# getreu/stringsext

Measured on AMD Instinct MI355X. Metric: GiB/s scanned, higher is better.
Workload: dtype u8

## Files before the change

include/stringsext_amd.h:

```cpp
#ifndef STRINGSEXT_AMD_H
#define STRINGSEXT_AMD_H
#include <stddef.h>
#include <stdint.h>

#ifdef __cplusplus
extern "C" {
#endif

#define SX_ABI_VERSION 4

enum {
    SX_OK = 0,
    SX_E_INVALID = -1,
    SX_E_NO_DEVICE = -2,
    SX_E_HIP = -3,
    SX_E_NOMEM = -4,
    SX_E_STATE = -5,
    SX_E_HALO = -6
};

enum {
    SX_ENC_X_USER_DEFINED = 0, SX_ENC_UTF8 = 1, SX_ENC_UTF16LE = 2, SX_ENC_UTF16BE = 3,
    SX_ENC_KOI8_R = 16, SX_ENC_IBM866 = 17, SX_ENC_ISO_8859_2 = 18, SX_ENC_ISO_8859_5 = 19,
    SX_ENC_ISO_8859_15 = 20, SX_ENC_WINDOWS_1251 = 21, SX_ENC_WINDOWS_1252 = 22,
// ... 171 lines not shown
                         sx_result** out, uint64_t* end_pos);
int sx_scan_shard(sx_ctx* ctx, const uint8_t* bytes, uint64_t buf_off, uint64_t buf_len,
                  uint64_t own_lo, uint64_t own_hi, const uint64_t* start_at,
                  uint64_t file_stream_off, int input_file_id, int reuse_runs,
                  sx_result** out, uint64_t* end_pos);
int sx_replay_shard_runs(sx_ctx* ctx, const uint8_t* bytes, uint64_t buf_off, uint64_t buf_len,
                         uint64_t own_lo, uint64_t own_hi, const uint64_t* start_at,
                         uint64_t file_stream_off, int input_file_id,
                         const sx_run* const* runs, const uint64_t* n_runs,
                         sx_result** out, uint64_t* end_pos);

typedef int (*sx_allgather_fn)(void* user, const void* send, uint64_t bytes, void* recv);
typedef int (*sx_shard_buffer_fn)(void* user, uint64_t lo, uint64_t hi, const void** ptr, int* is_device);
typedef int (*sx_shard_runs_fn)(void* user, const uint8_t* bytes, uint64_t buf_off, uint64_t buf_len,
                                const sx_run* const** runs, const uint64_t** n_runs);
void sx_shard_bounds(uint64_t file_len, int world, int rank, uint64_t* own_lo, uint64_t* own_hi);
int sx_scan_sharded(sx_ctx* ctx, int rank, int world, uint64_t file_len, uint64_t file_stream_off, int input_file_id,
                    uint64_t halo, sx_shard_buffer_fn get_buffer, void* buffer_user, sx_shard_runs_fn get_runs, void* runs_user,
                    sx_allgather_fn allgather, void* allgather_user, sx_result** out, uint64_t* counts, uint64_t* overflow);
int sx_shard_splice(const sx_finding* const* findings, const uint64_t* n_findings, const uint8_t* const* arenas,
                    const uint64_t* arena_lens, int world, uint64_t file_len, sx_result** out);
int sx_shard_splice_segs(const sx_finding* const* findings, const uint64_t* n_findings, const uint8_t* const* arenas,
                         const uint64_t* arena_lens, const uint32_t* n_segs_of_rank, int world, uint64_t file_len, sx_result** out);

#define SX_TRANSPORT_ID_BYTES 128
typedef struct sx_transport sx_transport;
int  sx_transport_rccl_id(uint8_t* id128);
int  sx_transport_rccl_create(sx_transport** out, int hip_device, int rank, int world, const uint8_t* id128);
void sx_transport_destroy(sx_transport* t);
const char* sx_transport_last_error(const sx_transport* t);
int  sx_transport_allgather(void* transport, const void* send, uint64_t bytes, void* recv);
int  sx_transport_gather(sx_transport* t, const sx_result* mine, int root, uint64_t file_len, sx_result** out);

int               sx_result_segment_device(const sx_result* r, uint64_t i, const void** d_records, uint64_t* n_findings,
                                           const uint8_t** d_arena, uint64_t* arena_len, int* packed, sx_segment_info* info);
uint64_t          sx_result_count(const sx_result* r);
uint64_t          sx_result_segments(const sx_result* r);
int               sx_result_segment(const sx_result* r, uint64_t index, const sx_finding** findings,
                                    uint64_t* n_findings, const uint8_t** arena, uint64_t* arena_len);
int               sx_result_segment_packed(const sx_result* r, uint64_t index, const void** findings, uint64_t* n_findings,
                                           const uint8_t** arena, uint64_t* arena_len, int* packed, sx_segment_info* info);
const sx_finding* sx_result_findings(const sx_result* r);
const uint8_t*    sx_result_arena(const sx_result* r, uint64_t* len);
void              sx_result_free(sx_result* r);

#define SX_OUTPUT_BOM "\xEF\xBB\xBF"
int sx_print_findings(const sx_ctx* ctx, const sx_result* r, int n_inputs, int radix,
                      int no_metadata, uint8_t** out, uint64_t* out_len);
int sx_print_findings_device(sx_ctx* ctx, const sx_result* r, int n_inputs, int radix, int no_metadata,
                             const uint8_t** d_text, uint64_t* text_len);

#define SX_SELECT_MAX_PATTERNS 16
#define SX_SELECT_MAX_PATTERN_BYTES 64
enum { SX_SELECT_ASCII_NOCASE = 1u,
       SX_SELECT_INVERT = 2u };
typedef struct sx_pattern { const uint8_t* bytes; uint32_t len; } sx_pattern;
int sx_result_select_device(sx_ctx* ctx, const sx_result* r, const sx_pattern* patterns, int n_patterns,
                            uint32_t flags, sx_result** out);

#define SX_SELECT_SET_MAX_PATTERNS      65536u
#define SX_SELECT_SET_MAX_PATTERN_BYTES 255u
#define SX_SELECT_SET_MAX_TOTAL_BYTES   (1u << 20)
typedef struct sx_select_set sx_select_set;
typedef struct sx_select_set_info {
    uint32_t n_patterns, states, classes, nocase;
    uint64_t table_bytes;
    uint32_t lds_states;
    uint32_t reserved;
} sx_select_set_info;
int  sx_select_set_create(sx_ctx* ctx, const sx_pattern* patterns, uint32_t n_patterns, uint32_t flags, sx_select_set** out);
int  sx_select_set_info_get(const sx_select_set* set, sx_select_set_info* out);
void sx_select_set_free(sx_select_set* set);
int  sx_result_select_set_device(sx_ctx* ctx, const sx_result* r, const sx_select_set* set, uint32_t flags, sx_result** out);

int  sx_get_stats(const sx_ctx* ctx, sx_stats* out);
void sx_free(void* p);

int sx_fill_background_device(sx_ctx* ctx, void* device_bytes, uint64_t first_byte_index,
                              uint64_t len, uint64_t seed);
int sx_device_alloc(sx_ctx* ctx, uint64_t bytes, void** device_ptr);
int sx_device_free(sx_ctx* ctx, void* device_ptr);
int sx_device_upload(sx_ctx* ctx, void* device_dst, const void* host_src, uint64_t bytes);
int sx_device_download(sx_ctx* ctx, void* host_dst, const void* device_src, uint64_t bytes);
int sx_device_read_bandwidth(sx_ctx* ctx, const void* device_bytes, uint64_t len, int repeats,
                             double* gbytes_per_s);

#ifdef __cplusplus
}
#endif
#endif
```

stringsext_amd/__init__.py:

```python
import ctypes as C
import os

_HERE = os.path.dirname(os.path.abspath(__file__))
LIB_PATH = os.environ.get("SX_LIB") or os.path.join(_HERE, "libstringsext_amd.so")

SX_OK, SX_E_INVALID, SX_E_NO_DEVICE, SX_E_HIP, SX_E_NOMEM, SX_E_STATE, SX_E_HALO = 0, -1, -2, -3, -4, -5, -6
SX_HOST_ONLY = -1
SX_OPT_GENERIC_KERNELS, SX_OPT_DEVICE_REPLAY, SX_OPT_HOST_REPLAY = 1, 2, 4
SX_OPT_NO_FUSED_SCAN = 64
SX_SELECT_MAX_PATTERNS, SX_SELECT_MAX_PATTERN_BYTES = 16, 64
SX_SELECT_ASCII_NOCASE, SX_SELECT_INVERT = 1, 2
SX_SELECT_SET_MAX_PATTERNS, SX_SELECT_SET_MAX_PATTERN_BYTES, SX_SELECT_SET_MAX_TOTAL_BYTES = 65536, 255, 1 << 20
SX_OPT_RESULT_ON_DEVICE = 32
ENC = {"x-user-defined": 0, "utf-8": 1, "utf-16le": 2, "utf-16be": 3, "koi8-r": 16, "ibm866": 17,
       "iso-8859-2": 18, "iso-8859-5": 19, "iso-8859-15": 20, "windows-1251": 21, "windows-1252": 22,
       "iso-8859-3": 23, "iso-8859-4": 24, "iso-8859-6": 25, "iso-8859-7": 26, "iso-8859-8": 27,
       "iso-8859-8-i": 28, "iso-8859-10": 29, "iso-8859-13": 30, "iso-8859-14": 31, "iso-8859-16": 32,
       "koi8-u": 33, "macintosh": 34, "windows-874": 35, "windows-1250": 36, "windows-1253": 37,
       "windows-1254": 38, "windows-1255": 39, "windows-1256": 40, "windows-1257": 41, "windows-1258": 42,
       "x-mac-cyrillic": 43, "big5": 64, "euc-jp": 65, "shift_jis": 66, "euc-kr": 67, "gb18030": 68, "gbk": 69, "replacement": 70}
PRECISION = {0: "Before", 1: "Exact", 2: "After"}

ABI_VERSION = 4
EXPORTS = ["sx_abi_version", "sx_create", "sx_destroy", "sx_last_error", "sx_scan", "sx_scan_device", "sx_reset",
           "sx_device_runs", "sx_device_runs_multi", "sx_replay_runs", "sx_scan_shard_device", "sx_scan_shard", "sx_replay_shard_runs",
           "sx_scan_stream", "sx_scan_file", "sx_missions_from_flags", "sx_parse_enc_opt", "sx_encoding_for_label", "sx_encoding_name",
           "sx_decoder_table", "sx_wave_classes", "sx_scan_classifier", "sx_result_segment_packed", "sx_wave_swar", "sx_wave_pair_codes2", "sx_wave_pair_codes", "sx_shard_bounds", "sx_scan_sharded", "sx_shard_splice", "sx_shard_splice_segs", "sx_transport_rccl_id", "sx_transport_rccl_create", "sx_transport_destroy", "sx_transport_last_error", "sx_transport_allgather", "sx_transport_gather",
           "sx_result_count", "sx_result_segments", "sx_result_segment", "sx_result_segment_device", "sx_result_findings", "sx_result_arena",
           "sx_result_free", "sx_print_findings", "sx_print_findings_device", "sx_result_select_device",
           "sx_select_set_create", "sx_select_set_info_get", "sx_select_set_free", "sx_result_select_set_device", "sx_get_stats", "sx_free", "sx_fill_background_device",
           "sx_device_alloc", "sx_device_free", "sx_device_upload", "sx_device_download",
           "sx_device_read_bandwidth"]


class Mission(C.Structure):
    _fields_ = [("mission_id", C.c_uint8), ("encoding", C.c_uint8), ("chars_min_nb", C.c_uint8),
                ("require_same_unicode_block", C.c_uint8), ("grep_char", C.c_int16),
                ("print_encoding_as_ascii", C.c_uint8), ("reserved", C.c_uint8),
                ("output_line_char_nb_max", C.c_uint32), ("af_lo", C.c_uint64), ("af_hi", C.c_uint64),
                ("ubf", C.c_uint64), ("counter_offset", C.c_uint64)]

    @classmethod
    def from_dict(cls, d):
        m = cls()
        m.mission_id = d["mission_id"]
        m.encoding = d["encoding"]
        m.chars_min_nb = d["chars_min_nb"]
        m.require_same_unicode_block = 1 if d["require_same_unicode_block"] else 0
        m.grep_char = -1 if d["grep_char"] is None else d["grep_char"]
        m.print_encoding_as_ascii = 1 if d["print_encoding_as_ascii"] else 0
        m.output_line_char_nb_max = d["output_line_char_nb_max"]
        m.af_lo = d["af"] & 0xFFFFFFFFFFFFFFFF
        m.af_hi = d["af"] >> 64
        m.ubf = d["ubf"]
        m.counter_offset = d["counter_offset"]
        return m

    def to_dict(self):
        return dict(mission_id=self.mission_id, encoding=self.encoding, chars_min_nb=self.chars_min_nb,
                    require_same_unicode_block=bool(self.require_same_unicode_block),
                    grep_char=None if self.grep_char < 0 else self.grep_char,
                    af=(self.af_hi << 64) | self.af_lo, ubf=self.ubf,
                    output_line_char_nb_max=self.output_line_char_nb_max, counter_offset=self.counter_offset,
                    print_encoding_as_ascii=bool(self.print_encoding_as_ascii))


class CliFlags(C.Structure):
    _fields_ = [("counter_offset", C.c_char_p), ("encodings", C.POINTER(C.c_char_p)), ("n_encodings", C.c_int),
                ("chars_min", C.c_char_p), ("same_unicode_block", C.c_int), ("ascii_filter", C.c_char_p),
                ("unicode_block_filter", C.c_char_p), ("grep_char", C.c_char_p), ("output_line_len", C.c_char_p)]


class EncOpt(C.Structure):
    _fields_ = [("has_name", C.c_int), ("name", C.c_char * 64), ("has_chars_min", C.c_int), ("chars_min", C.c_uint8),
                ("has_af", C.c_int), ("af_lo", C.c_uint64), ("af_hi", C.c_uint64), ("has_ubf", C.c_int), ("ubf", C.c_uint64),
                ("has_grep_char", C.c_int), ("grep_char", C.c_uint8)]


def missions_from_flags(encodings=(), chars_min=None, same_unicode_block=False, ascii_filter=None,
                        unicode_block_filter=None, grep_char=None, output_line_len=None, counter_offset=None):
    enc = [e.encode() for e in encodings]
    arr = (C.c_char_p * max(1, len(enc)))(*enc)
    b = lambda v: None if v is None else str(v).encode()
    f = CliFlags(b(counter_offset), arr, len(enc), b(chars_min), int(bool(same_unicode_block)), b(ascii_filter),
                 b(unicode_block_filter), b(grep_char), b(output_line_len))
    out = (Mission * 32)()
    n = C.c_int()
    err = C.create_string_buffer(512)
    L = lib()
    L.sx_missions_from_flags.argtypes = [C.POINTER(CliFlags), C.POINTER(Mission), C.c_int, C.POINTER(C.c_int), C.c_char_p, C.c_size_t]
    rc = L.sx_missions_from_flags(C.byref(f), out, 32, C.byref(n), err, 512)
    if rc != SX_OK:
        raise SxError(rc, err.value.decode())
    return [out[i].to_dict() for i in range(n.value)]


def encoding_name(enc):
    L = lib()
    L.sx_encoding_name.argtypes, L.sx_encoding_name.restype = [C.c_uint32], C.c_char_p
    s = L.sx_encoding_name(enc)
    return s.decode() if s else None


def decoder_table(enc):
    L = lib()
    L.sx_decoder_table.argtypes, L.sx_decoder_table.restype = [C.c_uint32, C.POINTER(C.c_uint64)], C.POINTER(C.c_uint16)
    n = C.c_uint64()
    t = L.sx_decoder_table(enc, C.byref(n))
    return (t, n.value) if n.value else None


def encoding_for_label(label):
    L = lib()
    L.sx_encoding_for_label.argtypes, L.sx_encoding_for_label.restype = [C.c_char_p], C.c_int
# ... 41 lines not shown
class Run(C.Structure):
    _fields_ = [("start", C.c_uint64), ("end", C.c_uint64), ("chars", C.c_uint64)]


class Stats(C.Structure):
    _fields_ = [("bytes_scanned", C.c_uint64), ("run_records", C.c_uint64), ("replay_bytes", C.c_uint64),
                ("findings", C.c_uint64), ("kernel_ms", C.c_double * 16), ("device_ms", C.c_double),
                ("h2d_ms", C.c_double), ("d2h_ms", C.c_double), ("replay_ms", C.c_double),
                ("total_ms", C.c_double), ("heavy_tiles", C.c_uint64), ("wave_windows", C.c_uint64),
                ("wave_count_ms", C.c_double), ("wave_write_ms", C.c_double), ("rescans", C.c_uint64), ("rescan_ms", C.c_double),
                ("wave_desc_overflows", C.c_uint64), ("seq_pieces", C.c_uint64),
                ("fast_regions", C.c_uint64), ("general_regions", C.c_uint64), ("wave_repairs", C.c_uint64),
                ("fused_ms", C.c_double), ("fused_launches", C.c_uint64), ("fused_mask", C.c_uint64)]


class Options(C.Structure):
    _fields_ = [("subchunk_bytes", C.c_uint32), ("record_capacity", C.c_uint32), ("replay_threads", C.c_uint32),
                ("flags", C.c_uint32)]


class SxError(RuntimeError):
    def __init__(self, code, msg):
        super().__init__(f"stringsext_amd error {code}: {msg}")
        self.code = code


_lib = None


def lib():
    global _lib
    if _lib is not None:
        return _lib
    if not os.path.exists(LIB_PATH):
        raise ImportError(f"{LIB_PATH} is missing: build it with `make -C stringsext_amd/csrc` "
                          "(or __graft_entry__.build()); there is no CPU fallback")
    L = C.CDLL(LIB_PATH)
    vp, u64, cp = C.c_void_p, C.c_uint64, C.c_char_p
    L.sx_abi_version.restype = C.c_int
    if L.sx_abi_version() != ABI_VERSION:
        raise ImportError(f"{LIB_PATH} has ABI version {L.sx_abi_version()}, this binding is written for {ABI_VERSION}: rebuild the library")
    L.sx_create.argtypes = [C.POINTER(vp), C.POINTER(Mission), C.c_int, C.c_int, C.POINTER(Options)]
    L.sx_destroy.argtypes = [vp]
    L.sx_last_error.restype = cp
    L.sx_last_error.argtypes = [vp]
    L.sx_scan.argtypes = [vp, cp, u64, C.c_int, C.c_int, C.POINTER(vp)]
    L.sx_scan_device.argtypes = [vp, vp, u64, C.c_int, C.c_int, C.POINTER(vp)]
    L.sx_reset.argtypes = [vp]
    L.sx_device_runs.argtypes = [vp, C.c_int, vp, u64, C.c_int, u64, C.POINTER(C.POINTER(Run)), C.POINTER(u64)]
    L.sx_device_runs_multi.argtypes = [vp, C.POINTER(C.c_int), C.c_int, vp, u64, C.c_int, C.POINTER(u64), C.POINTER(C.POINTER(Run)), C.POINTER(u64)]
    L.sx_replay_runs.argtypes = [vp, cp, u64, C.c_int, C.c_int, C.POINTER(C.POINTER(Run)), C.POINTER(u64),
                                 C.POINTER(vp)]
    pu64 = C.POINTER(u64)
    L.sx_scan_shard_device.argtypes = [vp, vp, u64, u64, u64, u64, pu64, u64, C.c_int, C.c_int, C.POINTER(vp), pu64]
    L.sx_scan_shard.argtypes = [vp, cp, u64, u64, u64, u64, pu64, u64, C.c_int, C.c_int, C.POINTER(vp), pu64]
    L.sx_replay_shard_runs.argtypes = [vp, cp, u64, u64, u64, u64, pu64, u64, C.c_int, C.POINTER(C.POINTER(Run)), pu64,
                                       C.POINTER(vp), pu64]
    L.sx_result_count.restype = u64
    L.sx_result_count.argtypes = [vp]
    L.sx_result_findings.restype = C.POINTER(Finding)
    L.sx_result_findings.argtypes = [vp]
    L.sx_result_arena.restype = C.POINTER(C.c_uint8)
    L.sx_result_arena.argtypes = [vp, C.POINTER(u64)]
    L.sx_result_free.argtypes = [vp]
    L.sx_result_segments.restype = u64
    L.sx_result_segments.argtypes = [vp]
    L.sx_result_segment.argtypes = [vp, u64, C.POINTER(C.POINTER(Finding)), C.POINTER(u64),
                                    C.POINTER(C.POINTER(C.c_uint8)), C.POINTER(u64)]
    L.sx_print_findings.argtypes = [vp, vp, C.c_int, C.c_int, C.c_int, C.POINTER(C.POINTER(C.c_uint8)),
                                    C.POINTER(u64)]
    L.sx_print_findings_device.argtypes = [vp, vp, C.c_int, C.c_int, C.c_int, C.POINTER(vp), C.POINTER(u64)]
    L.sx_result_select_device.argtypes = [vp, vp, C.POINTER(Pattern), C.c_int, C.c_uint32, C.POINTER(vp)]
    L.sx_select_set_create.argtypes = [vp, C.POINTER(Pattern), C.c_uint32, C.c_uint32, C.POINTER(vp)]
    L.sx_select_set_info_get.argtypes = [vp, C.POINTER(SelectSetInfo)]
    L.sx_select_set_free.argtypes, L.sx_select_set_free.restype = [vp], None
    L.sx_result_select_set_device.argtypes = [vp, vp, vp, C.c_uint32, C.POINTER(vp)]
    L.sx_get_stats.argtypes = [vp, C.POINTER(Stats)]
    L.sx_free.argtypes = [vp]
    L.sx_fill_background_device.argtypes = [vp, vp, u64, u64, u64]
    L.sx_device_alloc.argtypes = [vp, u64, C.POINTER(vp)]
    L.sx_device_free.argtypes = [vp, vp]
    L.sx_device_upload.argtypes = [vp, vp, cp, u64]
    L.sx_device_download.argtypes = [vp, vp, vp, u64]
    L.sx_device_read_bandwidth.argtypes = [vp, vp, u64, C.c_int, C.POINTER(C.c_double)]
    _lib = L
    return L


class Result:

    def __init__(self, scanner, handle):
        self._s, self.h = scanner, handle

    def __len__(self):
        return lib().sx_result_count(self.h)

    def raw(self):
        L = lib()
        n = L.sx_result_count(self.h)
        alen = C.c_uint64()
        ap = L.sx_result_arena(self.h, C.byref(alen))
        fp = L.sx_result_findings(self.h)
        if n and not fp:
            raise SxError(SX_E_INVALID, lib().sx_last_error(self._s.h).decode() or "result too large for one arena: use segments()")
        fb = C.string_at(fp, n * C.sizeof(Finding)) if n else b""
        return fb, (C.string_at(ap, alen.value) if alen.value and ap else b"")

    def segment_pointers(self):
        L = lib()
        out = []
        for i in range(L.sx_result_segments(self.h)):
            fp, n, ap, alen = C.POINTER(Finding)(), C.c_uint64(), C.POINTER(C.c_uint8)(), C.c_uint64()
            self._s._chk(L.sx_result_segment(self.h, i, C.byref(fp), C.byref(n), C.byref(ap), C.byref(alen)))
            out.append((fp, n.value, ap, alen.value))
        return out

    def finding_arrays(self):
        L = lib()
        out = []
        for i in range(L.sx_result_segments(self.h)):
            fp, n, ap, alen = C.POINTER(Finding)(), C.c_uint64(), C.POINTER(C.c_uint8)(), C.c_uint64()
            self._s._chk(L.sx_result_segment(self.h, i, C.byref(fp), C.byref(n), C.byref(ap), C.byref(alen)))
            out.append((fp, n.value))
        return out

    def packed_segments(self):
        L = lib()
        L.sx_result_segment_packed.argtypes = [C.c_void_p, C.c_uint64, C.POINTER(C.c_void_p), C.POINTER(C.c_uint64), C.POINTER(C.POINTER(C.c_uint8)),
                                               C.POINTER(C.c_uint64), C.POINTER(C.c_int), C.POINTER(SegmentInfo)]
        out = []
        for i in range(L.sx_result_segments(self.h)):
            fp, n, ap, alen, pk, info = C.c_void_p(), C.c_uint64(), C.POINTER(C.c_uint8)(), C.c_uint64(), C.c_int(), SegmentInfo()
            self._s._chk(L.sx_result_segment_packed(self.h, i, C.byref(fp), C.byref(n), C.byref(ap), C.byref(alen), C.byref(pk), C.byref(info)))
            recs = C.cast(fp, C.POINTER(Finding16 if pk.value else Finding))
            out.append((bool(pk.value), recs, n.value, C.string_at(ap, alen.value) if alen.value else b"", info))
        return out

    def device_segments(self):
        L = lib()
        L.sx_result_segment_device.argtypes = [C.c_void_p, C.c_uint64, C.POINTER(C.c_void_p), C.POINTER(C.c_uint64), C.POINTER(C.c_void_p),
                                               C.POINTER(C.c_uint64), C.POINTER(C.c_int), C.POINTER(SegmentInfo)]
        out = []
        for i in range(L.sx_result_segments(self.h)):
            fp, n, ap, alen, pk, info = C.c_void_p(), C.c_uint64(), C.c_void_p(), C.c_uint64(), C.c_int(), SegmentInfo()
            self._s._chk(L.sx_result_segment_device(self.h, i, C.byref(fp), C.byref(n), C.byref(ap), C.byref(alen), C.byref(pk), C.byref(info)))
            out.append((fp.value, n.value, ap.value, alen.value, bool(pk.value), info))
        return out

    def segments(self):
        L = lib()
        out = []
        for i in range(L.sx_result_segments(self.h)):
            fp, n, ap, alen = C.POINTER(Finding)(), C.c_uint64(), C.POINTER(C.c_uint8)(), C.c_uint64()
            self._s._chk(L.sx_result_segment(self.h, i, C.byref(fp), C.byref(n), C.byref(ap), C.byref(alen)))
            out.append((fp, n.value, C.string_at(ap, alen.value) if alen.value else b""))
        return out

    def findings(self):
        out = []
        for v, n, arena in self.segments():
            out += [dict(position=v[i].position, precision=PRECISION[v[i].precision],
                         s=arena[v[i].str_off:v[i].str_off + v[i].str_len].decode("utf-8"),
                         completes=bool(v[i].completes_previous), mission_id=v[i].mission_id,
                         file_id=v[i].input_file_id, slice_index=v[i].slice_index) for i in range(n)]
        return out

# ... 147 lines not shown
        return Result(self, r), list(ends)

    def device_runs(self, mission_index, dptr, length, stream_parity=0, min_chars=1, count_only=False):
        runs = C.POINTER(Run)()
        n = C.c_uint64()
        self._chk(lib().sx_device_runs(self.h, mission_index, dptr, length, stream_parity, min_chars,
                                       C.byref(runs), C.byref(n)))
        out = n.value if count_only else [(runs[i].start, runs[i].end, runs[i].chars) for i in range(n.value)]
        lib().sx_free(runs)
        return out

    def device_runs_multi(self, mission_indices, dptr, length, stream_parity=0, min_chars=None):
        n = len(mission_indices)
        idx = (C.c_int * n)(*mission_indices)
        mc = (C.c_uint64 * n)(*(min_chars if min_chars is not None else [1] * n))
        runs = (C.POINTER(Run) * n)()
        cnt = (C.c_uint64 * n)()
        self._chk(lib().sx_device_runs_multi(self.h, idx, n, dptr, length, stream_parity, mc, runs, cnt))
        out = []
        for i in range(n):
            out.append([(runs[i][j].start, runs[i][j].end, runs[i][j].chars) for j in range(cnt[i])])
            lib().sx_free(runs[i])
        return out

    def scan_file(self, path, chunk_bytes=0, file_id=1):
        results = []
        SINK = C.CFUNCTYPE(C.c_int, C.c_void_p, C.c_void_p)

        def sink(_user, handle):
            results.append(Result(self, C.c_void_p(handle)))
            return 0
        cb = SINK(sink)
        L = lib()
        L.sx_scan_file.argtypes = [C.c_void_p, C.c_char_p, C.c_uint64, C.c_int, SINK, C.c_void_p]
        self._chk(L.sx_scan_file(self.h, os.fsencode(path), chunk_bytes, file_id, cb, None))
        return results

    def scan_stream(self, readinto, chunk_bytes=0, file_id=1):
        results = []
        SINK = C.CFUNCTYPE(C.c_int, C.c_void_p, C.c_void_p)
        READ = C.CFUNCTYPE(C.c_int64, C.c_void_p, C.POINTER(C.c_uint8), C.c_uint64)

        def sink(_user, handle):
            results.append(Result(self, C.c_void_p(handle)))
            return 0

        def read(_user, dst, max_bytes):
            try:
                view = memoryview((C.c_uint8 * max_bytes).from_address(C.addressof(dst.contents))).cast("B")
                return int(readinto(view) or 0)
            except Exception:
                return -1
        cb, rd = SINK(sink), READ(read)
        L = lib()
        L.sx_scan_stream.argtypes = [C.c_void_p, READ, C.c_void_p, C.c_uint64, C.c_int, SINK, C.c_void_p]
        self._chk(L.sx_scan_stream(self.h, rd, None, chunk_bytes, file_id, cb, None))
        return results

    def reset(self):
        self._chk(lib().sx_reset(self.h))

    def stats(self):
        s = Stats()
        self._chk(lib().sx_get_stats(self.h, C.byref(s)))
        return s

    def alloc(self, nbytes):
        p = C.c_void_p()
        self._chk(lib().sx_device_alloc(self.h, nbytes, C.byref(p)))
        return p

    def free(self, dptr):
        self._chk(lib().sx_device_free(self.h, dptr))

    def upload(self, dptr, data):
        data = bytes(data)
        self._chk(lib().sx_device_upload(self.h, dptr, data, len(data)))

    def download(self, dptr, nbytes):
        b = C.create_string_buffer(nbytes)
        self._chk(lib().sx_device_download(self.h, b, dptr, nbytes))
        return b.raw

    def fill_background(self, dptr, first_index, nbytes, seed=0x5EED5EED5EED5EED):
        self._chk(lib().sx_fill_background_device(self.h, dptr, first_index, nbytes, seed))

    def read_bandwidth(self, dptr, nbytes, repeats=5):
        g = C.c_double()
        self._chk(lib().sx_device_read_bandwidth(self.h, dptr, nbytes, repeats, C.byref(g)))
        return g.value

    def close(self):
        if self.h:
            lib().sx_destroy(self.h)
            self.h = None

    def __del__(self):
        try:
            self.close()
        except Exception:
            pass


OUTPUT_BOM = b"\xEF\xBB\xBF"
```

stringsext_amd/csrc/sx_api.cpp:

```cpp
#include "sx_ctx.hpp"
#include "sx_print_core.hpp"
#include "sx_select_core.hpp"
#include "sx_selset_build.hpp"
#include "sx_selset_core.hpp"

using namespace sx;

struct sx_select_set {
    int device = 0;
    uint8_t* mem = nullptr;
    SelsetDevice dev{};
    sx_select_set_info info{};
};

namespace sx {
PinnedPool::Block PinnedPool::take(size_t bytes) {
    {
        std::lock_guard<std::mutex> g(mu);
        size_t best = free_blocks.size();
        for (size_t i = 0; i < free_blocks.size(); i++)
            if (free_blocks[i].cap >= bytes && (best == free_blocks.size() || free_blocks[i].cap < free_blocks[best].cap)) best = i;
        if (best < free_blocks.size() && free_blocks[best].cap <= 4 * bytes + (4u << 20)) {
            Block b = free_blocks[best];
            free_blocks.erase(free_blocks.begin() + (long)best);
            return b;
        }
    }
    Block b;
    const size_t cap = bytes + bytes / 8 + (1u << 20);
    if (hipHostMalloc(&b.p, cap, hipHostMallocNonCoherent) != hipSuccess) { b.p = nullptr; return b; }
    b.cap = cap;
    return b;
}
void PinnedPool::give(Block b) {
    if (!b.p) return;
    std::lock_guard<std::mutex> g(mu);
    free_blocks.push_back(b);
    if (free_blocks.size() > 40) {
        size_t m = 0;
        for (size_t i = 1; i < free_blocks.size(); i++) if (free_blocks[i].cap < free_blocks[m].cap) m = i;
        (void)hipHostFree(free_blocks[m].p);
        free_blocks.erase(free_blocks.begin() + (long)m);
    }
}
PinnedPool::~PinnedPool() { for (Block& b : free_blocks) (void)hipHostFree(b.p); }
}

namespace {
std::string g_create_error;
}

namespace sx {

double g_tl_t0 = 0;
int g_tl_on = 0;

double now_ms() {
    using namespace std::chrono;
    return duration<double, std::milli>(steady_clock::now().time_since_epoch()).count();
}


int ensure_pinned(sx_ctx* ctx, uint64_t bytes) {
    if (ctx->h_pin_cap >= bytes) return SX_OK;
    if (ctx->h_pin) HIP_TRY(ctx, hipHostFree(ctx->h_pin));
    ctx->h_pin = nullptr; ctx->h_pin_cap = 0;
    bytes += bytes / 4 + (1u << 20);
    unsigned flags = hipHostMallocNonCoherent;
    if (ctx->sw.pin_flags >= 0) flags = (unsigned)ctx->sw.pin_flags;
    HIP_TRY(ctx, hipHostMalloc((void**)&ctx->h_pin, bytes, flags));
    ctx->h_pin_cap = bytes;
    return SX_OK;
}
int read_back_async(sx_ctx* ctx, hipStream_t s, void* pinned_dst, const void* dev_src, size_t bytes) {
    if (ctx->sw.small_copy && bytes <= (1u << 20) && ((((uintptr_t)pinned_dst | (uintptr_t)dev_src | bytes) & 3) == 0))
        HIP_TRY(ctx, launch_small_copy(pinned_dst, dev_src, bytes, s));
    else HIP_TRY(ctx, hipMemcpyAsync(pinned_dst, dev_src, bytes, hipMemcpyDeviceToHost, s));
    return SX_OK;
}
int read_back_sync(sx_ctx* ctx, MissionDev& d, hipStream_t s, void* host_dst, const void* dev_src, size_t bytes) {
    if (!ctx->sw.small_copy || bytes > kSmallReadBytes || ((((uintptr_t)dev_src | bytes) & 3) != 0)) {
        HIP_TRY(ctx, hipMemcpyAsync(host_dst, dev_src, bytes, hipMemcpyDeviceToHost, s));
        HIP_TRY(ctx, hipStreamSynchronize(s));
        return SX_OK;
    }
    if (!d.h_small) HIP_TRY(ctx, hipHostMalloc((void**)&d.h_small, kSmallReadBytes, hipHostMallocDefault));
    HIP_TRY(ctx, launch_small_copy(d.h_small, dev_src, bytes, s));
    HIP_TRY(ctx, hipStreamSynchronize(s));
    memcpy(host_dst, d.h_small, bytes);
    return SX_OK;
}
int ensure_pinned2(sx_ctx* ctx, uint64_t bytes) {
    if (ctx->h_pin2_cap >= bytes) return SX_OK;
    if (ctx->h_pin2) HIP_TRY(ctx, hipHostFree(ctx->h_pin2));
    ctx->h_pin2 = nullptr; ctx->h_pin2_cap = 0;
    bytes += bytes / 4 + (1u << 20);
    HIP_TRY(ctx, hipHostMalloc((void**)&ctx->h_pin2, bytes, hipHostMallocNonCoherent));
    ctx->h_pin2_cap = bytes;
    return SX_OK;
}
int ensure_scratch(sx_ctx* ctx, uint64_t bytes) {
    std::lock_guard<std::recursive_mutex> g(ctx->grow_mu);
    if (ctx->d_scratch_cap >= bytes) return SX_OK;
    if (ctx->merge_async) { const int rc = merge_drain(ctx); if (rc != SX_OK) return rc; }
    if (ctx->d_scratch) HIP_TRY(ctx, hipFree(ctx->d_scratch));
    ctx->d_scratch = nullptr; ctx->d_scratch_cap = 0;
    bytes += bytes / 4 + (1u << 20);
    HIP_TRY(ctx, hipMalloc((void**)&ctx->d_scratch, bytes));
    ctx->d_scratch_cap = bytes;
    return SX_OK;
}

int ensure_capacity(sx_ctx* ctx, ScanSlot& s, uint32_t cap) {
    if (s.capacity >= cap) return SX_OK;
    if (s.d_recs) HIP_TRY(ctx, hipFree(s.d_recs));
    s.d_recs = nullptr; s.capacity = 0;
    HIP_TRY(ctx, hipMalloc((void**)&s.d_recs, (size_t)cap * sizeof(DevRun)));
    s.capacity = cap;
    return SX_OK;
}

int ensure_cache(sx_ctx* ctx, uint64_t bytes) {
    if (ctx->d_cache_cap >= bytes) return SX_OK;
    if (ctx->d_cache) HIP_TRY(ctx, hipFree(ctx->d_cache));
    ctx->d_cache = nullptr; ctx->d_cache_cap = 0;
    HIP_TRY(ctx, hipMalloc((void**)&ctx->d_cache, bytes));
    ctx->d_cache_cap = bytes;
    return SX_OK;
}
int ensure_rp(sx_ctx* ctx, MissionDev& d, int slot, uint64_t bytes) {
    if (d.d_rp_cap[slot] >= bytes) return SX_OK;
    std::lock_guard<std::recursive_mutex> g(ctx->grow_mu);
    if (ctx->merge_async) { const int rc = merge_drain(ctx); if (rc != SX_OK) return rc; }
    if (d.d_rp[slot]) HIP_TRY(ctx, hipFree(d.d_rp[slot]));
    d.d_rp[slot] = nullptr; d.d_rp_cap[slot] = 0;
    bytes += bytes / 4 + 4096;
    HIP_TRY(ctx, hipMalloc(&d.d_rp[slot], bytes));
    d.d_rp_cap[slot] = bytes;
    return SX_OK;
}


unsigned usable_cpus() {
    unsigned n = std::thread::hardware_concurrency();
    if (n < 1) n = 1;
    if (FILE* f = fopen("/sys/fs/cgroup/cpu.max", "r")) {
        char a[64] = { 0 };
        unsigned long long period = 0;
        if (fscanf(f, "%63s %llu", a, &period) == 2 && strcmp(a, "max") != 0 && period > 0) {
            const unsigned long long quota = strtoull(a, nullptr, 10);
            const unsigned q = (unsigned)((quota + period - 1) / period);
            if (q >= 1 && q < n) n = q;
        }
        fclose(f);
    }
    return n;
}

unsigned replay_threads(const sx_ctx* ctx) {
    unsigned n = ctx->opt.replay_threads ? ctx->opt.replay_threads
                                         : std::min(std::thread::hardware_concurrency(), 4 * usable_cpus());
    if (ctx->sw.replay_threads) n = (unsigned)ctx->sw.replay_threads;
    if (n < 1) n = 1;
    return n > 256 ? 256 : n;
}


void begin_call(sx_ctx* ctx) {
    memset(&ctx->stats, 0, sizeof ctx->stats);
    ctx->err.clear();
    ctx->sharded_call = false;
    ctx->dev_epoch->fetch_add(1);
}

static int fetch_to_host(sx_result* r, MissionFindings& s) {
    if (!s.dev_only) return SX_OK;
    if (!s.keep_on_device || !s.dev_epoch_ref || s.dev_epoch_ref->load() != s.dev_epoch) return SX_E_STATE;
    const size_t bytes = s.ext_nf * s.rec_size() + s.ext_na;
    PinnedPool::Block blk = r->r.pool ? r->r.pool->take(bytes + 64) : PinnedPool::Block{};
    if (!blk.p) return SX_E_NOMEM;
    if (hipMemcpy(blk.p, s.dev_copy, bytes, hipMemcpyDeviceToHost) != hipSuccess) { r->r.pool->give(blk); return SX_E_HIP; }
// ... 135 lines not shown
        for (ScanSlot& s : d.slot) {
            if ((e = hipEventCreate(&s.ev0)) != hipSuccess) return fail("hipEventCreate", e);
            if ((e = hipEventCreate(&s.ev1)) != hipSuccess) return fail("hipEventCreate", e);
            if ((e = hipEventCreateWithFlags(&s.ev_free, hipEventDisableTiming)) != hipSuccess) return fail("hipEventCreate", e);
            if ((e = hipMalloc((void**)&s.d_counters, kCounterWords * sizeof(uint32_t))) != hipSuccess) return fail("hipMalloc", e);
            if ((e = hipMalloc((void**)&s.d_recs, (size_t)cap * sizeof(DevRun))) != hipSuccess) return fail("hipMalloc", e);
            s.capacity = cap;
        }
    }
    for (size_t k = 0; k < ctx->dev.size(); k++) {
        size_t n_words = 0;
        if (const uint16_t* t = decoder_table(ctx->missions[k].c.encoding, &n_words)) {
            if ((e = hipMalloc((void**)&ctx->dev[k].d_table, n_words * 2)) != hipSuccess) return fail("hipMalloc", e);
            if ((e = hipMemcpy(ctx->dev[k].d_table, t, n_words * 2, hipMemcpyHostToDevice)) != hipSuccess) return fail("hipMemcpy", e);
        }
        const std::vector<uint32_t>& pl = ctx->missions[k].pair_lut;
        if (!pl.empty()) {
            if ((e = hipMalloc((void**)&ctx->dev[k].d_pair_lut, pl.size() * 4)) != hipSuccess) return fail("hipMalloc", e);
            if ((e = hipMemcpy(ctx->dev[k].d_pair_lut, pl.data(), pl.size() * 4, hipMemcpyHostToDevice)) != hipSuccess) return fail("hipMemcpy", e);
        }
    }
    *out = ctx;
    return SX_OK;
}

void sx_destroy(sx_ctx* ctx) {
    if (!ctx) return;
    ctx->dev_epoch->fetch_add(1);
    for (auto& e : ctx->select_epoch) e->fetch_add(1);
    if (!ctx->host_only && ctx->device >= 0) {
        (void)hipSetDevice(ctx->device);
        for (auto& d : ctx->dev) {
            if (d.stream) (void)hipStreamSynchronize(d.stream);
            if (d.stream_b) (void)hipStreamSynchronize(d.stream_b);
            for (ScanSlot& s : d.slot) {
                if (s.d_recs) (void)hipFree(s.d_recs);
                if (s.d_cnt) (void)hipFree(s.d_cnt);
                if (s.d_grid) (void)hipFree(s.d_grid);
                if (s.d_packed) (void)hipFree(s.d_packed);
                if (s.d_counters) (void)hipFree(s.d_counters);
                if (s.ev0) (void)hipEventDestroy(s.ev0);
                if (s.ev1) (void)hipEventDestroy(s.ev1);
                if (s.ev_free) (void)hipEventDestroy(s.ev_free);
            }
            if (d.d_table) (void)hipFree(d.d_table);
            if (d.d_pair_lut) (void)hipFree(d.d_pair_lut);
            if (d.d_wave_lut) (void)hipFree(d.d_wave_lut);
            if (d.d_wave_pairs) (void)hipFree(d.d_wave_pairs);
            if (d.d_wave_pairs2) (void)hipFree(d.d_wave_pairs2);
            for (void* q : d.d_rp) if (q) (void)hipFree(q);
            if (d.h_runs) (void)hipHostFree(d.h_runs);
            if (d.ev_runs) (void)hipEventDestroy(d.ev_runs);
            if (d.stream_w) (void)hipStreamDestroy(d.stream_w);
            if (d.h_tot) (void)hipHostFree(d.h_tot);
            if (d.h_small) (void)hipHostFree(d.h_small);
            for (hipEvent_t e : d.wave_ev) if (e) (void)hipEventDestroy(e);
            if (d.stream && d.stream != ctx->scan_stream) (void)hipStreamDestroy(d.stream);
        }
        for (int i = 0; i < 2; i++) {
            if (ctx->ing_pin[i]) (void)hipHostFree(ctx->ing_pin[i]);
            if (ctx->ing_dev[i]) (void)hipFree(ctx->ing_dev[i]);
        }
        if (ctx->copy_stream) (void)hipStreamDestroy(ctx->copy_stream);
        if (ctx->d2h_stream) (void)hipStreamDestroy(ctx->d2h_stream);
        if (ctx->scan_stream) (void)hipStreamDestroy(ctx->scan_stream);
        if (ctx->d_cache) (void)hipFree(ctx->d_cache);
        if (ctx->post_stream) (void)hipStreamDestroy(ctx->post_stream);
        if (ctx->merge_copy_stream) (void)hipStreamDestroy(ctx->merge_copy_stream);
        if (ctx->d_merge) (void)hipFree(ctx->d_merge);
        if (ctx->d_result) (void)hipFree(ctx->d_result);
        if (ctx->d_result_up) (void)hipFree(ctx->d_result_up);
        if (ctx->d_text) (void)hipFree(ctx->d_text);
        if (ctx->d_print_scratch) (void)hipFree(ctx->d_print_scratch);
        if (ctx->d_print_missions) (void)hipFree(ctx->d_print_missions);
        for (uint8_t* p : ctx->d_select) if (p) (void)hipFree(p);
        if (ctx->d_select_scratch) (void)hipFree(ctx->d_select_scratch);
        if (ctx->d_select_scratch2) (void)hipFree(ctx->d_select_scratch2);
        for (hipEvent_t e : ctx->merge_ev) if (e) (void)hipEventDestroy(e);
        if (ctx->ev_interleaved) (void)hipEventDestroy(ctx->ev_interleaved);
        if (ctx->d_input) (void)hipFree(ctx->d_input);
        if (ctx->d_scratch) (void)hipFree(ctx->d_scratch);
        if (ctx->h_pin) (void)hipHostFree(ctx->h_pin);
        if (ctx->h_pin2) (void)hipHostFree(ctx->h_pin2);
    }
    delete ctx;
}

const char* sx_last_error(const sx_ctx* ctx) { return ctx ? ctx->err.c_str() : g_create_error.c_str(); }

int sx_reset(sx_ctx* ctx) {
    if (!ctx) return SX_E_INVALID;
    for (size_t k = 0; k < ctx->missions.size(); k++) ctx->states[k].reset(ctx->missions[k]);
    ctx->shard_runs_valid = false;
    return SX_OK;
}


int sx_device_runs(sx_ctx* ctx, int mission_index, const void* device_bytes, uint64_t len, int stream_parity,
                   uint64_t min_chars, sx_run** runs, uint64_t* n_runs) {
    if (!ctx || !runs || !n_runs || mission_index < 0 || (size_t)mission_index >= ctx->missions.size()) return SX_E_INVALID;
    begin_call(ctx);
    ctx->sw.scan_warm = Switches::from_env().scan_warm;
    if (ctx->host_only) { ctx->err = "host-only context: no device scan"; return SX_E_STATE; }
    if ((uintptr_t)device_bytes & 15) { ctx->err = "device_bytes must be 16-byte aligned"; return SX_E_INVALID; }
    if (ctx->missions[(size_t)mission_index].host_sequential()) { ctx->err = "an ISO-2022-JP mission has no stage A (one sequential pass on the host)"; return SX_E_INVALID; }
    HIP_TRY(ctx, hipSetDevice(ctx->device));
    std::vector<RunList> out;
    ctx->shard_runs_valid = false;
    int rc = device_runs(ctx, { mission_index }, (const uint8_t*)device_bytes, len, { (uint32_t)(stream_parity & 1) },
                         { min_chars }, &out);
    if (rc != SX_OK) return rc;
    HIP_TRY(ctx, out[0].wait());
    *n_runs = out[0].size();
    *runs = (sx_run*)malloc(sizeof(sx_run) * (out[0].size() ? out[0].size() : 1));
    if (!*runs) return SX_E_NOMEM;
    memcpy(*runs, out[0].data(), sizeof(sx_run) * out[0].size());
    return SX_OK;
}

int sx_device_runs_multi(sx_ctx* ctx, const int* mission_indices, int n, const void* device_bytes, uint64_t len, int stream_parity,
                         const uint64_t* min_chars, sx_run** runs, uint64_t* n_runs) {
    if (!ctx || !mission_indices || n <= 0 || !min_chars || !runs || !n_runs) return SX_E_INVALID;
    begin_call(ctx);
    if (ctx->host_only) { ctx->err = "host-only context: no device scan"; return SX_E_STATE; }
    if ((uintptr_t)device_bytes & 15) { ctx->err = "device_bytes must be 16-byte aligned"; return SX_E_INVALID; }
    std::vector<int> which; std::vector<uint32_t> par; std::vector<uint64_t> mc;
    for (int i = 0; i < n; i++) {
        const int k = mission_indices[i];
        if (k < 0 || (size_t)k >= ctx->missions.size() || std::find(which.begin(), which.end(), k) != which.end()) { ctx->err = "bad mission index"; return SX_E_INVALID; }
        if (ctx->missions[(size_t)k].host_sequential()) { ctx->err = "an ISO-2022-JP mission has no stage A (one sequential pass on the host)"; return SX_E_INVALID; }
        which.push_back(k); par.push_back((uint32_t)(stream_parity & 1)); mc.push_back(min_chars[i]);
        runs[i] = nullptr; n_runs[i] = 0;
    }
    HIP_TRY(ctx, hipSetDevice(ctx->device));
    std::vector<RunList> out;
    ctx->shard_runs_valid = false;
    int rc = device_runs(ctx, which, (const uint8_t*)device_bytes, len, par, mc, &out);
    if (rc != SX_OK) return rc;
    for (int i = 0; i < n; i++) {
        if (!out[(size_t)i].own.empty()) out[(size_t)i].use_own();
        HIP_TRY(ctx, out[(size_t)i].wait());
        n_runs[i] = out[(size_t)i].size();
        runs[i] = (sx_run*)malloc(sizeof(sx_run) * (n_runs[i] ? n_runs[i] : 1));
        if (!runs[i]) { for (int j = 0; j < i; j++) { free(runs[j]); runs[j] = nullptr; } return SX_E_NOMEM; }
        memcpy(runs[i], out[(size_t)i].data(), sizeof(sx_run) * n_runs[i]);
    }
    return SX_OK;
}

int sx_replay_runs(sx_ctx* ctx, const uint8_t* bytes, uint64_t len, int input_file_id, int is_last_input_buffer,
                   const sx_run* const* runs, const uint64_t* n_runs, sx_result** out) {
    if (!ctx || !out || (!bytes && len) || !runs || !n_runs) return SX_E_INVALID;
    begin_call(ctx);
    std::vector<RunList> r(ctx->missions.size());
    for (size_t k = 0; k < r.size(); k++) r[k].assign(runs[k], runs[k] + n_runs[k]);
    HostBytes view(bytes ? bytes : (const uint8_t*)"");
    ResultHolder res;
    std::vector<uint32_t> entry;
    int rc = set_entry_params(ctx, true, bytes, nullptr, len, 0, &entry);
    if (rc != SX_OK) return rc;
    rc = replay_all(ctx, view, whole_chunk_job(ctx, len, input_file_id, is_last_input_buffer != 0), r, &res.r->r, nullptr);
    if (rc == SX_OK) *out = res.release();
    return rc;
}


// ... 313 lines not shown
    { const int rc = selset_build(patterns, n_patterns, flags, &T, &err); if (rc != SX_OK) { ctx->set_err("pattern set: " + err); return rc; } }
    if (ctx->host_only) { ctx->set_err("host-only context: no device for the pattern set"); return SX_E_STATE; }
    HIP_TRY(ctx, hipSetDevice(ctx->device));
    const size_t table = (T.next.size() + 15) / 16 * 16;
    uint8_t* mem = nullptr;
    if (hipMalloc((void**)&mem, sizeof T.map + table) != hipSuccess) {
        (void)hipGetLastError();
        ctx->set_err("pattern set: no device memory for " + std::to_string(sizeof T.map + table) + " bytes of table");
        return SX_E_NOMEM;
    }
    hipError_t e = hipMemcpy(mem, T.map, sizeof T.map, hipMemcpyHostToDevice);
    if (e == hipSuccess) e = hipMemcpy(mem + sizeof T.map, T.next.data(), T.next.size(), hipMemcpyHostToDevice);
    if (e != hipSuccess) { (void)hipFree(mem); ctx->set_err(std::string("hipMemcpy: ") + hipGetErrorString(e)); return SX_E_HIP; }
    sx_select_set* set = new (std::nothrow) sx_select_set;
    if (!set) { (void)hipFree(mem); return SX_E_NOMEM; }
    set->device = ctx->device; set->mem = mem;
    set->dev = SelsetDevice{ mem, mem + sizeof T.map, T.states, T.classes, T.lds_states, T.matched, T.entry_bytes, 0 };
    set->info = sx_select_set_info{ T.n_patterns, T.states, T.classes, T.nocase, (uint64_t)T.next.size(), T.lds_states, 0 };
    *out = set;
    return SX_OK;
}

int sx_select_set_info_get(const sx_select_set* set, sx_select_set_info* out) {
    if (!set || !out) return SX_E_INVALID;
    *out = set->info;
    return SX_OK;
}

void sx_select_set_free(sx_select_set* set) {
    if (!set) return;
    (void)hipFree(set->mem);
    delete set;
}

int sx_result_select_set_device(sx_ctx* ctx, const sx_result* r, const sx_select_set* set, uint32_t flags, sx_result** out) {
    if (out) *out = nullptr;
    if (!ctx || !r || !set || !out) return SX_E_INVALID;
    if (flags & ~(uint32_t)SX_SELECT_INVERT) { ctx->set_err("a pattern set is selected with SX_SELECT_INVERT or no flag: the fold is compiled into the set"); return SX_E_INVALID; }
    if (ctx->host_only) { ctx->set_err("host-only context: no device selection"); return SX_E_STATE; }
    if (set->device != ctx->device) { ctx->set_err("the pattern set lies on another device"); return SX_E_INVALID; }
    return select_on_device(ctx, r, nullptr, 0, &set->dev, flags, out);
}

int sx_get_stats(const sx_ctx* ctx, sx_stats* out) {
    if (!ctx || !out) return SX_E_INVALID;
    *out = ctx->stats;
    return SX_OK;
}

void sx_free(void* p) { free(p); }

int sx_fill_background_device(sx_ctx* ctx, void* device_bytes, uint64_t first_byte_index, uint64_t len, uint64_t seed) {
    if (!ctx || ctx->host_only) return SX_E_STATE;
    HIP_TRY(ctx, hipSetDevice(ctx->device));
    HIP_TRY(ctx, launch_fill_background((uint8_t*)device_bytes, first_byte_index, len, seed, ctx->dev[0].stream_b));
    HIP_TRY(ctx, hipStreamSynchronize(ctx->dev[0].stream_b));
    return SX_OK;
}

int sx_device_alloc(sx_ctx* ctx, uint64_t bytes, void** device_ptr) {
    if (!ctx || ctx->host_only || !device_ptr) return SX_E_STATE;
    HIP_TRY(ctx, hipSetDevice(ctx->device));
    HIP_TRY(ctx, hipMalloc(device_ptr, bytes ? bytes : 1));
    return SX_OK;
}
int sx_device_free(sx_ctx* ctx, void* device_ptr) {
    if (!ctx || ctx->host_only) return SX_E_STATE;
    HIP_TRY(ctx, hipFree(device_ptr));
    return SX_OK;
}
int sx_device_upload(sx_ctx* ctx, void* device_dst, const void* host_src, uint64_t bytes) {
    if (!ctx || ctx->host_only) return SX_E_STATE;
    HIP_TRY(ctx, hipSetDevice(ctx->device));
    HIP_TRY(ctx, hipMemcpy(device_dst, host_src, bytes, hipMemcpyHostToDevice));
    return SX_OK;
}
int sx_device_download(sx_ctx* ctx, void* host_dst, const void* device_src, uint64_t bytes) {
    if (!ctx || ctx->host_only) return SX_E_STATE;
    HIP_TRY(ctx, hipSetDevice(ctx->device));
    HIP_TRY(ctx, hipMemcpy(host_dst, device_src, bytes, hipMemcpyDeviceToHost));
    return SX_OK;
}

int sx_device_read_bandwidth(sx_ctx* ctx, const void* device_bytes, uint64_t len, int repeats, double* gbytes_per_s) {
    if (!ctx || ctx->host_only || !gbytes_per_s || repeats == 0) return SX_E_STATE;
    HIP_TRY(ctx, hipSetDevice(ctx->device));
    MissionDev& d = ctx->dev[0];
    uint64_t* d_out = nullptr;
    HIP_TRY(ctx, hipMalloc((void**)&d_out, 8));
    HIP_TRY(ctx, hipMemsetAsync(d_out, 0, 8, d.stream));
    const uint32_t sub = repeats < 0 ? (ctx->opt.subchunk_bytes ? ctx->opt.subchunk_bytes : 256u * 1024u) : 0u;
    if (repeats < 0) repeats = -repeats;
    HIP_TRY(ctx, launch_read_sum((const uint8_t*)device_bytes, len, d_out, d.stream, sub, ctx->sw.probe_rot));
    float best = 1e30f;
    for (int i = 0; i < repeats; i++) {
        HIP_TRY(ctx, hipEventRecord(d.slot[0].ev0, d.stream));
        HIP_TRY(ctx, launch_read_sum((const uint8_t*)device_bytes, len, d_out, d.stream, sub, ctx->sw.probe_rot));
        HIP_TRY(ctx, hipEventRecord(d.slot[0].ev1, d.stream));
        HIP_TRY(ctx, hipStreamSynchronize(d.stream));
        float ms = 0;
        HIP_TRY(ctx, hipEventElapsedTime(&ms, d.slot[0].ev0, d.slot[0].ev1));
        if (ms < best) best = ms;
    }
    (void)hipFree(d_out);
    *gbytes_per_s = (double)(len / 16 * 16) / (best * 1e-3) / 1e9;
    return SX_OK;
}

}
```

stringsext_amd/csrc/sx_ctx.hpp:

```cpp
#pragma once
#include <hip/hip_runtime_api.h>
#include <stdio.h>
#include <stdlib.h>
#include <string.h>
#include <errno.h>
#include <fcntl.h>
#include <sys/mman.h>
#include <sys/stat.h>
#include <unistd.h>

#include <algorithm>
#include <atomic>
#include <chrono>
#include <condition_variable>
#include <deque>
#include <functional>
#include <mutex>
#include <string>
#include <thread>
#include <unordered_map>
#include <vector>

#include "sx_host.hpp"
#include "sx_switches.hpp"
// ... 73 lines not shown
    uint32_t* d_wave_pairs = nullptr;
    uint32_t* d_wave_pairs2 = nullptr;
    uint8_t* d_wave_lut = nullptr;
    sx_run* h_runs = nullptr; uint64_t h_runs_cap = 0;
    hipEvent_t ev_runs = nullptr;
    void* d_rp[12] = { nullptr, nullptr, nullptr, nullptr, nullptr, nullptr, nullptr, nullptr, nullptr, nullptr, nullptr, nullptr };
    uint64_t d_rp_cap[12] = { 0, 0, 0, 0, 0, 0, 0, 0, 0, 0, 0, 0 };
    hipStream_t stream_w = nullptr;
    uint64_t* h_tot = nullptr;
    const uint32_t* grid_of_scan = nullptr; uint32_t grid_sub = 0; const uint8_t* grid_data = nullptr; uint64_t grid_len = 0;
    uint8_t* h_small = nullptr;
    std::vector<hipEvent_t> wave_ev;
};


}

struct sx_result {
    sx::Result r;
};

struct sx_ctx {
    std::shared_ptr<sx::PinnedPool> pool = std::make_shared<sx::PinnedPool>();
    std::shared_ptr<std::atomic<uint64_t>> dev_epoch = std::make_shared<std::atomic<uint64_t>>(0);
    std::vector<sx::Mission> missions;
    std::vector<sx::ScannerState> states;
    std::vector<sx::MissionDev> dev;
    bool host_only = false;
    bool sharded_call = false, single_piece = true;
    int device = -1;
    sx_options opt{};
    sx::Switches sw;
    std::string err;
    sx_stats stats{};
    hipStream_t scan_stream = nullptr, post_stream = nullptr;
    uint8_t* d_cache = nullptr;
    uint64_t d_cache_cap = 0;
    hipStream_t merge_copy_stream = nullptr;
    hipEvent_t merge_ev[3] = { nullptr, nullptr, nullptr };
    uint8_t* d_merge = nullptr; uint64_t d_merge_cap = 0, merge_out_room = 0, merge_n_out = 0;
    uint8_t* d_result = nullptr; uint64_t d_result_cap = 0;
    uint8_t* d_result_up = nullptr; uint64_t d_result_up_cap = 0;
    uint8_t* d_text = nullptr; uint64_t d_text_cap = 0;
    uint8_t* d_print_scratch = nullptr; uint64_t d_print_scratch_cap = 0;
    uint8_t* d_print_missions = nullptr;
    uint8_t* d_select[2] = { nullptr, nullptr }; uint64_t d_select_cap[2] = { 0, 0 };
    std::shared_ptr<std::atomic<uint64_t>> select_epoch[2] = { std::make_shared<std::atomic<uint64_t>>(0), std::make_shared<std::atomic<uint64_t>>(0) };
    uint64_t select_calls = 0;
    uint8_t* d_select_scratch = nullptr; uint64_t d_select_scratch_cap = 0;
    uint8_t* d_select_scratch2 = nullptr; uint64_t d_select_scratch2_cap = 0;
    bool merge_async = false;
    bool merge_copy_pending[2] = { false, false };
    uint64_t merge_parts = 0;
    uint64_t merged_out_bytes = 0;
    double out_density = 0;
    hipEvent_t ev_interleaved = nullptr;
    std::atomic<bool> interleave_pending{ false };
    std::mutex mu;
    std::mutex err_mu;
    std::recursive_mutex grow_mu;
    void set_err(std::string text) { std::lock_guard<std::mutex> g(err_mu); err = std::move(text); }
    unsigned n_cus = 256, scan_blocks_per_cu = 8;
    hipStream_t copy_stream = nullptr;
    hipStream_t d2h_stream = nullptr;
    uint8_t* ing_pin[2] = { nullptr, nullptr };
    uint8_t* ing_dev[2] = { nullptr, nullptr };
    uint64_t ing_cap = 0, ing_dev_cap = 0;
    uint32_t region_cap = 64;
    std::vector<uint32_t> dense;
    uint8_t* d_input = nullptr;
    uint64_t d_input_cap = 0;
    uint64_t ondemand_fetches = 0;
    std::vector<uint64_t> last_runs;
    std::vector<char> wave_pred;
    std::vector<double> wave_density;
    std::vector<char> wave_off;
    std::vector<sx::RunList> shard_runs;
    bool shard_runs_valid = false;
    uint64_t shard_runs_off = 0, shard_runs_len = 0;
    const void* shard_runs_ptr = nullptr;
    uint8_t* h_pin = nullptr;   uint64_t h_pin_cap = 0;
    uint8_t* h_pin2 = nullptr;  uint64_t h_pin2_cap = 0;
    uint8_t* d_scratch = nullptr; uint64_t d_scratch_cap = 0;
};

#define HIP_TRY(ctx, expr)                                                                     \
    do {                                                                                       \
        hipError_t e_ = (expr);                                                                \
        if (e_ != hipSuccess) {                                                                \
            (ctx)->set_err(std::string(#expr) + ": " + hipGetErrorString(e_));                 \
            return SX_E_HIP;                                                                   \
        }                                                                                      \
    } while (0)

namespace sx {

class SparseDeviceBytes : public ByteView {
public:
    SparseDeviceBytes(sx_ctx* ctx, const uint8_t* d_base, uint64_t len = 0) : ctx_(ctx), d_base_(d_base), len_(len) {}
    void add(uint64_t lo, uint64_t hi, const uint8_t* p) { segs_.push_back({ lo, hi, p }); }
    void add_copy(uint64_t lo, uint64_t hi, const uint8_t* p) {
        owned_.emplace_back(p, p + (hi - lo));
        segs_.push_back({ lo, hi, owned_.back().data() });
    }
    bool empty() const { return segs_.empty(); }
    const uint8_t* span(uint64_t off, size_t n, size_t* hint) override {
        size_t a = *hint < segs_.size() ? *hint : 0;
        if (!(a < segs_.size() && segs_[a].lo <= off)) a = 0;
        size_t steps = 0;
        while (a < segs_.size() && segs_[a].hi <= off && steps < 8) { a++; steps++; }
        if (!(a < segs_.size() && segs_[a].lo <= off && off < segs_[a].hi)) {
            size_t lo = 0, hi = segs_.size();
            while (lo < hi) {
                size_t mid = (lo + hi) / 2;
                if (segs_[mid].hi <= off) lo = mid + 1; else hi = mid;
            }
            a = lo;
        }
        if (a < segs_.size() && segs_[a].lo <= off && off + n <= segs_[a].hi) { *hint = a; return segs_[a].p + (off - segs_[a].lo); }
        std::lock_guard<std::mutex> g(mu_);
        if (len_) {
            const uint64_t b = off / kBlock;
            if (off + n <= std::min<uint64_t>(len_, (b + 1) * kBlock)) {
                auto it = blocks_.find(b);
                if (it == blocks_.end()) {
                    const uint64_t lo = b * kBlock, hi = std::min<uint64_t>(len_, lo + kBlock);
                    std::vector<uint8_t> v((size_t)(hi - lo));
                    if (hipMemcpy(v.data(), d_base_ + lo, (size_t)(hi - lo), hipMemcpyDeviceToHost) != hipSuccess) memset(v.data(), 0, v.size());
                    ctx_->ondemand_fetches++;
                    it = blocks_.emplace(b, std::move(v)).first;
                }
                return it->second.data() + (off - b * kBlock);
            }
        }
        extra_.emplace_back(n);
        if (hipMemcpy(extra_.back().data(), d_base_ + off, n, hipMemcpyDeviceToHost) != hipSuccess)
            memset(extra_.back().data(), 0, n);
        ctx_->ondemand_fetches++;
        return extra_.back().data();
    }

private:
    struct Seg { uint64_t lo, hi; const uint8_t* p; };
    sx_ctx* ctx_;
    const uint8_t* d_base_;
    uint64_t len_ = 0;
    static constexpr uint64_t kBlock = 65536;
    std::unordered_map<uint64_t, std::vector<uint8_t>> blocks_;
    std::vector<Seg> segs_;
    std::deque<std::vector<uint8_t>> extra_, owned_;
    std::mutex mu_;
};

int ensure_pinned(sx_ctx* ctx, uint64_t bytes);
int ensure_pinned2(sx_ctx* ctx, uint64_t bytes);
int read_back_sync(sx_ctx* ctx, sx::MissionDev& d, hipStream_t s, void* host_dst, const void* dev_src, size_t bytes);
int read_back_async(sx_ctx* ctx, hipStream_t s, void* pinned_dst, const void* dev_src, size_t bytes);
int ensure_scratch(sx_ctx* ctx, uint64_t bytes);
int ensure_capacity(sx_ctx* ctx, ScanSlot& s, uint32_t cap);
int ensure_rp(sx_ctx* ctx, MissionDev& d, int slot, uint64_t bytes);
int ensure_cache(sx_ctx* ctx, uint64_t bytes);
unsigned usable_cpus();
unsigned replay_threads(const sx_ctx* ctx);
void begin_call(sx_ctx* ctx);

ScanParams scan_params(const sx_ctx* ctx, int mission, const ScanSlot& s, const uint8_t* d_bytes, uint64_t len,
                       uint32_t parity, uint64_t min_chars);
int stage_a_launch(sx_ctx* ctx, const std::vector<int>& which, const uint8_t* d_bytes, uint64_t len,
                   const std::vector<uint32_t>& parity, const std::vector<uint64_t>& min_chars, int si);
struct ReplayJob;
int ensure_copy_stream(sx_ctx* ctx);
bool result_stays_on_device(const sx_ctx* ctx, const ReplayJob& job);
int merge_drain(sx_ctx* ctx);
int stage_a_finish(sx_ctx* ctx, const std::vector<int>& which, const uint8_t* d_bytes, uint64_t len,
                   const std::vector<uint32_t>& parity, const std::vector<uint64_t>& min_chars, int si,
                   std::vector<RunList>* out, bool cut_into_pieces = false, const ReplayJob* wave_job = nullptr);
int device_runs(sx_ctx* ctx, const std::vector<int>& which, const uint8_t* d_bytes, uint64_t len,
                const std::vector<uint32_t>& parity, const std::vector<uint64_t>& min_chars,
                std::vector<RunList>* out);

struct ReplayJob {
    uint64_t len = 0;
    int file_id = -1;
    bool is_last = false;
    std::vector<uint64_t> lo;
    uint64_t hi = 0;
    std::vector<char> entry_exact;
    std::vector<uint64_t> consumed0, stream0;
    bool commit_state = true;
    uint32_t slice_base = 0;
    const uint8_t* d_bytes = nullptr;
};




struct PreReplayed {
    std::vector<char> done;
    std::vector<MissionFindings> per;
    std::vector<uint64_t> ends;
    explicit PreReplayed(size_t nm) : done(nm, 0), per(nm), ends(nm, 0) {}
};


constexpr int SX_WAVE_FALLBACK = 1001;
constexpr int SX_NEED_RUNS = 1002;
bool wave_replay_wanted(const sx_ctx* ctx, const ReplayJob& job, size_t k, size_t n_runs, uint64_t heavy_tiles = 0);
int wave_replay_mission(sx_ctx* ctx, size_t k, ByteView& view, const ReplayJob& job, MissionFindings* out, uint64_t* end_pos,
                        uint64_t defer_min_bytes, bool own_stream = false);
bool device_replay_wanted(const sx_ctx* ctx, const ReplayJob& job, size_t k, size_t n_runs);
int device_replay_mission(sx_ctx* ctx, size_t k, ByteView& view, const ReplayJob& job, const RunList& runs,
                          MissionFindings* out, uint64_t* end_pos, uint64_t defer_min_bytes);
int replay_all(sx_ctx* ctx, ByteView& bytes, const ReplayJob& job, const std::vector<RunList>& runs,
               Result* into, uint64_t* end_pos, PreReplayed* pre = nullptr);
ReplayJob whole_chunk_job(sx_ctx* ctx, uint64_t len, int file_id, bool is_last);
int download_for_replay(sx_ctx* ctx, const uint8_t* d_bytes, uint64_t len,
                        const std::vector<RunList>* runs_opt, SparseDeviceBytes* view,
                        const ReplayJob& job, const std::vector<char>* skip = nullptr,
                        bool* used_base = nullptr);

struct ResultHolder {
    sx_result* r = new sx_result();
    ~ResultHolder() { delete r; }
    sx_result* release() { sx_result* x = r; r = nullptr; return x; }
};

int set_entry_params(sx_ctx* ctx, bool carried_state_is_entry, const uint8_t* host_bytes, const uint8_t* d_bytes, uint64_t len,
                     uint64_t stream_off, std::vector<uint32_t>* parity);
int scan_common(sx_ctx* ctx, const uint8_t* host_bytes, const uint8_t* d_bytes, uint64_t len, int file_id,
                int is_last, sx_result** out, uint32_t slice_base0 = 0, sx_result* append_to = nullptr);
int shard_common(sx_ctx* ctx, const uint8_t* host_bytes, const uint8_t* d_bytes,
                 const sx_run* const* given_runs, const uint64_t* given_n, uint64_t buf_off, uint64_t buf_len,
                 uint64_t own_lo, uint64_t own_hi, const uint64_t* start_at, uint64_t file_stream_off, int file_id,
                 int reuse_runs, sx_result** out, uint64_t* end_pos);
int stream_core(sx_ctx* ctx, sx_read_fn read, void* read_user, uint64_t chunk_bytes, int input_file_id,
                sx_result_fn sink, void* sink_user, sx_result* accumulate, int is_last_at_eof,
                const uint8_t* direct = nullptr, uint64_t direct_len = 0);

}
```

stringsext_amd/csrc/sx_device.hpp:

```cpp
#pragma once
#include <cstdlib>
#include <hip/hip_runtime_api.h>
#include <stdint.h>

#include "../../include/stringsext_amd.h"

namespace sx {

constexpr uint32_t kTileBytes = 1024;

struct DevRun {
    uint64_t start;
    uint32_t len;
    uint32_t chars_flags;
};
constexpr uint32_t kRecStartOpen = 0x80000000u;
constexpr uint32_t kRecEndOpen = 0x40000000u;
constexpr uint32_t kRecCharsMask = 0x3FFFFFFFu;
constexpr uint32_t kRecInvalidLen = 0xFFFFFFFFu, kRecInvalidFlags = 0xFFFFFFFFu;

constexpr uint32_t kStatBase = 32, kStatShards = 16, kStatStride = 32, kCounterWords = kStatBase + kStatShards * kStatStride;

enum ClassifierKind : uint32_t {
    kClsSingleByteLut = 0,
// ... 130 lines not shown
    const uint8_t* lut;
    const uint16_t* table;
    const uint32_t* pairs;
    uint32_t encoding;
    uint32_t entry_skip;
    uint32_t *wave_nf, *wave_nb, *wave_in, *wave_out;
    uint32_t* wave_grid;
    const uint64_t *wave_fbase, *wave_abase;
    uint64_t f_sub, a_sub;
    sx_finding* findings;
    uint8_t* arena;
    uint32_t packed;
    uint32_t str_off_base;
    uint64_t v0, v1;
    uint32_t* desc;
    uint32_t desc_cap;
    WvSwar swar;
    const uint32_t* pairs2;
    uint64_t* lead_set;
    uint64_t ubf;
    int32_t grep_char;
    uint32_t redo, use_entry;
    uint32_t same;
};
size_t wave_scratch_bytes(uint64_t n_waves);
hipError_t launch_wave_count(const WaveParams& P, uint64_t v0, uint64_t v1, uint64_t* fbase, uint64_t* abase, uint64_t* totals,
                             void* scratch, size_t scratch_bytes, hipStream_t stream);
hipError_t launch_wave_write(const WaveParams& P, uint64_t v0, uint64_t v1, hipStream_t stream);
hipError_t launch_wave_emit(const WaveParams& P, uint64_t v0, uint64_t v1, hipStream_t stream);

hipError_t merge_findings_device_part(const sx_finding* const* f, const uint8_t* const* a, const uint64_t* nf, const uint64_t* nb,
                                      const uint32_t* off0, int n_missions, void* out, void* scratch, size_t scratch_bytes,
                                      hipStream_t stream, int packed = 0, int ordered = 0);
bool merge_part_can_pack(uint64_t n, int n_missions);
hipError_t launch_slab_cuts(const ReplayParams& P, uint32_t n_slabs, uint64_t* idx, uint64_t* hi, hipStream_t stream);
hipError_t launch_merge_cuts(const sx_finding* f, uint64_t n, uint64_t nb, const uint64_t* cuts, uint32_t n_cuts, uint64_t* idx,
                             uint64_t* off, hipStream_t stream);
size_t merge_findings_scratch_bytes(uint64_t n_findings, int n_missions, int ordered = 0);
size_t order_strings_scratch_bytes(uint64_t n);
hipError_t order_part_strings(void* recs, uint64_t n, int packed, const uint64_t* src, uint8_t* arena, void* scratch, size_t scratch_bytes,
                              hipStream_t stream);
struct PrintParams;
size_t print_scratch_bytes(uint64_t n);
hipError_t print_measure(const PrintParams& P, void* scratch, size_t scratch_bytes, hipStream_t stream, const uint64_t** wbase, const uint64_t** total);
hipError_t print_write(const PrintParams& P, hipStream_t stream);
struct SelectParams;
struct SelsetDevice;
size_t select_scratch_bytes(uint64_t n);
hipError_t selset_launch_match(const SelectParams& P, const SelsetDevice& set, uint64_t waves, hipStream_t stream);
hipError_t select_measure(SelectParams* P, const SelsetDevice* set, void* scratch, size_t scratch_bytes, hipStream_t stream, const uint32_t** count, const uint64_t** bytes);
size_t select_place_scratch_bytes(uint64_t n_sel);
hipError_t select_place(const SelectParams& P, void* out_recs, uint64_t n_sel, uint8_t* out_arena, void* scratch, size_t scratch_bytes, hipStream_t stream);
hipError_t launch_copy_bytes(void* dst, const void* src, uint64_t bytes, uint32_t workgroups, hipStream_t stream, int threads, bool nontemporal);
hipError_t launch_small_copy(void* pinned_dst, const void* dev_src, size_t bytes, hipStream_t stream);

size_t sort_scratch_bytes(uint32_t n);
hipError_t sort_records(DevRun* recs, uint32_t n, uint64_t max_key, void* scratch, size_t scratch_bytes, hipStream_t stream, bool timing);

size_t compact_scratch_bytes(uint64_t n_regions);
hipError_t invalidate_region_slack(DevRun* recs, const uint32_t* counts, uint64_t n_regions, uint32_t region_cap, hipStream_t stream);
hipError_t compact_regions(const DevRun* recs, const uint32_t* counts, uint64_t n_regions, uint32_t region_cap, DevRun* out,
                           uint32_t* total, void* scratch, size_t scratch_bytes, hipStream_t stream);

size_t merge_scratch_bytes(uint32_t n);
hipError_t merge_sorted_records(const DevRun* recs, uint32_t n, uint64_t min_chars, void* scratch, size_t scratch_bytes,
                                sx_run* out, uint32_t* out_count, hipStream_t stream);

hipError_t launch_scan(ClassifierKind kind, const ScanParams& p, hipStream_t stream);
constexpr int kFusedMax = 3;
struct FusedParams {
    ScanParams m[kFusedMax];
    const uint8_t* data;
    uint64_t len;
    uint32_t subchunk;
    uint32_t fsh[kFusedMax][4];
    uint32_t cand_f[kFusedMax];
    uint32_t pf_zero[kFusedMax];
};
int fused_slot_of(ClassifierKind kind, const ScanParams& p);
hipError_t launch_scan_fused(const FusedParams& fp, uint32_t used, hipStream_t stream, int prefilter_override);
hipError_t launch_fill_background(uint8_t* dst, uint64_t first_index, uint64_t len, uint64_t seed,
                                  hipStream_t stream);
hipError_t launch_read_sum(const uint8_t* src, uint64_t len, uint64_t* out, hipStream_t stream, uint32_t subchunk = 0, uint32_t rot = 0);
hipError_t launch_gather(const uint8_t* src, uint8_t* dst, const uint64_t* seg_src, const uint64_t* seg_dst,
                         const uint32_t* seg_len, uint32_t n, hipStream_t stream);

}
```

stringsext_amd/csrc/sx_kernels.hip:

```cpp
#include "sx_scan_core.hpp"

namespace sx {

template <class CLS, bool NEEDS_LUT>
__global__ __launch_bounds__(256) __attribute__((amdgpu_waves_per_eu(NEEDS_LUT ? 6 : 7))) void scan_kernel(const ScanParams p) {
    __shared__ __attribute__((aligned(16))) uint8_t lds_lut[512];
    if (NEEDS_LUT) {
        lds_lut[threadIdx.x] = p.lut[threadIdx.x];
        lds_lut[threadIdx.x + 256] = p.lut[threadIdx.x + 256];
        __syncthreads();
    }
    const u32 lane = lane_id();
    if (p.wave_prio) __builtin_amdgcn_s_setprio(3);
    CLS cls;
    cls.init(p, lds_lut);
    Emitter em{ p.recs, p.counters, p.capacity, 0u, 0u, p.region_cap, 0u, p.region_counts };

    for (bool first_round = true;; first_round = false) {
    u64 wave;
    if (p.persistent) {
        u32 w = 0;
        if (lane == 0) w = atomicAdd(p.counters + 3, 1u);
        wave = uniform(w);
    } else {
// ... 559 lines not shown
        if (p.n_ranges <= 2) return launch_t<SingleByteRanges<2>, false>(p, stream);
        if (p.n_ranges <= 4) return launch_t<SingleByteRanges<4>, false>(p, stream);
        return launch_t<SingleByteRanges<6>, false>(p, stream);
    default: break;
    }
    return hipErrorInvalidValue;
}

SX_DEV u64 mix64(u64 z) {
    z = (z ^ (z >> 30)) * 0xBF58476D1CE4E5B9ull;
    z = (z ^ (z >> 27)) * 0x94D049BB133111EBull;
    return z ^ (z >> 31);
}

__global__ __launch_bounds__(256) void fill_kernel(uint8_t* dst, u64 first, u64 len, u64 seed) {
    u64 w0 = first >> 3, w1 = (first + len + 7) >> 3;
    u64 stride = (u64)gridDim.x * blockDim.x;
    for (u64 w = w0 + (u64)blockIdx.x * blockDim.x + threadIdx.x; w < w1; w += stride) {
        u64 v = mix64(seed + (w + 1) * 0x9E3779B97F4A7C15ull);
        u64 i0 = w << 3;
        if (i0 >= first && i0 + 8 <= first + len && (((uintptr_t)(dst + (i0 - first))) & 7) == 0) {
            *(u64*)(dst + (i0 - first)) = v;
        } else {
            for (int k = 0; k < 8; k++) {
                u64 i = i0 + k;
                if (i >= first && i < first + len) dst[i - first] = (uint8_t)(v >> (8 * k));
            }
        }
    }
}

hipError_t launch_fill_background(uint8_t* dst, u64 first, u64 len, u64 seed, hipStream_t stream) {
    if (len == 0) return hipSuccess;
    hipLaunchKernelGGL(fill_kernel, dim3(256 * 16), dim3(256), 0, stream, dst, first, len, seed);
    return hipGetLastError();
}

__global__ __launch_bounds__(256) void read_sum_kernel(const u32x4* src, u64 n16, u64* out) {
    u64 stride = (u64)gridDim.x * blockDim.x;
    u32 acc = 0;
    for (u64 i = (u64)blockIdx.x * blockDim.x + threadIdx.x; i < n16; i += stride) {
        u32x4 v = __builtin_nontemporal_load(src + i);
        acc += v.x ^ v.y ^ v.z ^ v.w;
    }
    if (acc == 0x12345678u) atomicAdd((unsigned long long*)out, 1ull);
}

__global__ __launch_bounds__(256) void read_subchunk_kernel(const uint8_t* data, u64 len, u32 subchunk, u64* out, u32 rot) {
    const u32 lane = lane_id();
    const u64 wave = (u64)blockIdx.x * 4u + uniform(threadIdx.x >> 6);
    const u64 sub_start = wave * (u64)subchunk;
    if (sub_start >= len) return;
    const u64 sub_end = sub_start + subchunk < len ? sub_start + subchunk : len;
    const uint8_t* base_ptr = data + sub_start;
    const u32 base_lo = uniform((u32)(uintptr_t)base_ptr), base_hi = uniform((u32)((uintptr_t)base_ptr >> 32));
    const __amdgpu_buffer_rsrc_t rsrc = __builtin_amdgcn_make_buffer_rsrc(
        (void*)(((u64)base_hi << 32) | base_lo), 0, (int)uniform((u32)(sub_end - sub_start)), 0x00020000);
    const int n_tiles = (int)((sub_end - sub_start) / kTileBytes);
    const u32 span = (u32)n_tiles * kTileBytes;
    u32 o0 = rot && n_tiles ? (u32)((wave * rot) % (u64)n_tiles) * kTileBytes : 0u;
    auto wrap = [&](u32 o) { return o >= span ? o - span : o; };
    u32x4 cur = __builtin_amdgcn_raw_buffer_load_b128(rsrc, (int)(o0 + lane * 16u), 0, 0);
    u32x4 nxt = __builtin_amdgcn_raw_buffer_load_b128(rsrc, (int)(wrap(o0 + kTileBytes) + lane * 16u), 0, 0);
    u32 acc = 0, off = wrap(o0 + 2 * kTileBytes);
    for (int t = 0; t < n_tiles; t++) {
        u32x4 nn = __builtin_amdgcn_raw_buffer_load_b128(rsrc, (int)(off + lane * 16u), 0, 0);
        acc += cur.x ^ cur.y ^ cur.z ^ cur.w;
        cur = nxt; nxt = nn; off = wrap(off + kTileBytes);
    }
    if (acc == 0x12345678u) atomicAdd((unsigned long long*)out, 1ull);
}

hipError_t launch_read_sum(const uint8_t* src, u64 len, u64* out, hipStream_t stream, uint32_t subchunk, uint32_t rot) {
    if (subchunk) {
        u64 waves = (len + subchunk - 1) / subchunk;
        const dim3 grid((unsigned)((waves + 3) / 4));
        hipLaunchKernelGGL(read_subchunk_kernel, grid, dim3(256), 0, stream, src, len, subchunk, out, (u32)rot);
    } else {
        hipLaunchKernelGGL(read_sum_kernel, dim3(256 * 8), dim3(256), 0, stream, (const u32x4*)src, len / 16, out);
    }
    return hipGetLastError();
}

__global__ __launch_bounds__(256) void gather_kernel(const uint8_t* src, uint8_t* dst, const u64* seg_src,
                                                     const u64* seg_dst, const u32* seg_len, u32 n) {
    u32 wave = (blockIdx.x * 256u + threadIdx.x) >> 6, lane = threadIdx.x & 63u;
    u32 nw = (gridDim.x * 256u) >> 6;
    for (u32 i = wave; i < n; i += nw) {
        const uint8_t* s = src + seg_src[i];
        uint8_t* d = dst + seg_dst[i];
        u32 l = seg_len[i];
        for (u32 k = lane; k < l; k += 64) d[k] = s[k];
    }
}

hipError_t launch_gather(const uint8_t* src, uint8_t* dst, const u64* seg_src, const u64* seg_dst,
                         const u32* seg_len, u32 n, hipStream_t stream) {
    if (n == 0) return hipSuccess;
    u32 blocks = (n + 3) / 4;
    if (blocks > 256 * 8) blocks = 256 * 8;
    hipLaunchKernelGGL(gather_kernel, dim3(blocks), dim3(256), 0, stream, src, dst, seg_src, seg_dst, seg_len, n);
    return hipGetLastError();
}

}
```

stringsext_amd/csrc/sx_schedule.cpp:

```cpp
#include "sx_ctx.hpp"
#include <thread>

using namespace sx;

namespace sx {

uint64_t piece_bytes(const sx_ctx* ctx, uint64_t len) {
    uint64_t piece = 0;
    bool halves = false;
    if (ctx->sw.piece_mib >= 0) piece = (uint64_t)ctx->sw.piece_mib << 20;
    else if (len >= (16ull << 30) && ctx->missions.size() >= 2 && !(ctx->opt.flags & (SX_OPT_NO_FUSED_SCAN | SX_OPT_MISSION_STREAMS | SX_OPT_RESULT_ON_DEVICE))) {
        piece = ((len / 100) * 50 + kInputBufLen - 1) / kInputBufLen * kInputBufLen;
        halves = true;
    }
    if (piece == 0 || (!halves && len < 2 * piece)) return len;
    for (const Mission& m : ctx->missions) if (m.is_dbcs()) return len;
    return piece / kInputBufLen * kInputBufLen;
}

static uint64_t seq_piece_bytes(const sx_ctx* ctx, uint64_t len) {
    uint64_t piece = 0;
    if (ctx->sw.seq_piece_kib >= 0) {
        piece = (uint64_t)ctx->sw.seq_piece_kib << 10;
        if (piece == 0) return len;
    } else if (ctx->sw.seq_piece_mib >= 0) {
        piece = (uint64_t)ctx->sw.seq_piece_mib << 20;
        if (piece == 0) return len;
    } else {
        if (ctx->opt.flags & SX_OPT_RESULT_ON_DEVICE) return len;
        if (ctx->missions.size() < 2 || ctx->out_density <= 0) return len;
        const double out = ctx->out_density * (double)len;
        if (out < 4.0 * (double)(1ull << 30)) return len;
        const uint64_t n = (uint64_t)(out / (2.25 * (double)(1ull << 30))) + 1;
        piece = std::max<uint64_t>((len + n - 1) / n, 1ull << 30);
    }
    piece = std::max<uint64_t>((piece + kInputBufLen - 1) / kInputBufLen, 2) * kInputBufLen;
    return len < 2 * piece ? len : piece;
}

static int entry_param(sx_ctx* ctx, size_t k, const Decoder* carried, const uint8_t* host_bytes, const uint8_t* d_bytes,
                       uint64_t len, uint64_t stream_off, uint32_t* out, uint32_t* out_replay = nullptr) {
    const Mission& m = ctx->missions[k];
    *out = (uint32_t)(stream_off & 1);
    if (out_replay) *out_replay = 0;
    if (!m.is_dbcs()) return SX_OK;
    *out = 0;
    if (!carried || carried->idle() || len == 0) return SX_OK;
    uint8_t first[8] = { 0, 0, 0, 0, 0, 0, 0, 0 };
    const uint64_t n = std::min<uint64_t>(8, len);
    if (host_bytes) memcpy(first, host_bytes, n);
    else HIP_TRY(ctx, hipMemcpy(first, d_bytes, n, hipMemcpyDeviceToHost));
    *out = carried->entry_skip_scan(first, n);
    if (out_replay) *out_replay = carried->entry_skip(first, n);
    if (ctx->sw.debug_entry) { const DDecoder& dd = const_cast<Decoder*>(carried)->raw(); fprintf(stderr, "[sx] entry mission %zu: dlead %02x gb2 %02x gb3 %02x rq_n %u first %02x %02x -> scan %u replay %u\n", k, dd.dlead, dd.gb2, dd.gb3, dd.rq_n, first[0], first[1], *out, out_replay ? *out_replay : 0u); }
    return SX_OK;
}
int set_entry_params(sx_ctx* ctx, bool carried_state_is_entry, const uint8_t* host_bytes, const uint8_t* d_bytes, uint64_t len,
                     uint64_t stream_off, std::vector<uint32_t>* parity) {
    parity->clear();
    for (size_t k = 0; k < ctx->missions.size(); k++) {
        uint32_t ep = 0, ep_replay = 0;
        int rc = entry_param(ctx, k, carried_state_is_entry ? &ctx->states[k].decoder : nullptr, host_bytes, d_bytes, len,
                             stream_off, &ep, &ep_replay);
        if (rc != SX_OK) return rc;
        parity->push_back(ep);
        ctx->missions[k].buf_entry_skip = ctx->missions[k].is_dbcs() ? ep_replay : 0u;
    }
    return SX_OK;
}

void mission_order(sx_ctx* ctx, std::vector<int>* out) {
    const size_t nm = ctx->missions.size();
    std::vector<int>& order = *out;
    order.resize(nm);
    for (size_t k = 0; k < nm; k++) order[k] = (int)k;
    if (ctx->last_runs.size() != nm) return;
    std::stable_sort(order.begin(), order.end(), [&](int x, int y) { return ctx->last_runs[(size_t)x] > ctx->last_runs[(size_t)y]; });
    const int mode = ctx->sw.busiest_last;
    if (mode) std::reverse(order.begin(), order.end());
    if (mode == 2 && nm >= 3) std::swap(order[nm - 1], order[nm - 2]);
}

int sync_streams_and_return(sx_ctx* ctx, int rc) {
    ctx->merge_async = false;
    (void)merge_drain(ctx);
    for (auto& d : ctx->dev) { (void)hipStreamSynchronize(d.stream); (void)hipStreamSynchronize(d.stream_b); }
    return rc;
}

struct BufferScan {
    const uint8_t* host_bytes = nullptr;
    const uint8_t* d_bytes = nullptr;
    uint64_t len = 0;
    std::vector<int> order;
    std::vector<uint32_t> parity;
    std::vector<uint64_t> minc;
    int slot = 0;
    std::unique_ptr<SparseDeviceBytes> base_view;
    bool whole = false;
    bool skip_scan(const sx_ctx* ctx, size_t k) const {
        return whole && len >= 2 * kInputBufLen && k < ctx->wave_pred.size() && ctx->wave_pred[k] && ctx->missions[k].wave_ok && !ctx->sw.wave_keep_scan
               && ctx->sw.wave_replay != 0;
    }
    bool none_scanned(const sx_ctx* ctx) const {
        if (not_scanned.size() != ctx->missions.size()) return false;
        for (char c : not_scanned) if (!c) return false;
        return true;
    }

    int fetch_base(sx_ctx* ctx) {
        base_view.reset();
        if (host_bytes) return SX_OK;
        base_view.reset(new SparseDeviceBytes(ctx, d_bytes, len));
        if (none_scanned(ctx)) return SX_OK;
        ReplayJob none;
        return download_for_replay(ctx, d_bytes, len, nullptr, base_view.get(), none);
    }
    std::vector<char> not_scanned;
    int launch(sx_ctx* ctx) {
        not_scanned.assign(ctx->missions.size(), 0);
        std::vector<int> ks; std::vector<uint32_t> par; std::vector<uint64_t> mc;
        for (int k : order) {
            if (ctx->missions[(size_t)k].host_sequential() || skip_scan(ctx, (size_t)k)) { not_scanned[(size_t)k] = 1; continue; }
            ks.push_back(k); par.push_back(parity[(size_t)k]); mc.push_back(minc[(size_t)k]);
        }
        return ks.empty() ? SX_OK : stage_a_launch(ctx, ks, d_bytes, len, par, mc, slot);
    }
    int finish_and_replay(sx_ctx* ctx, const ReplayJob& job, const std::function<int()>& after_last_finish,
                          std::vector<RunList>* runs, Result* into, uint64_t* ends) {
        const size_t nm = ctx->missions.size();
        runs->assign(nm, RunList{});
        HostBytes host_view(host_bytes ? host_bytes : (const uint8_t*)"");
        ByteView& early_view = host_bytes ? (ByteView&)host_view : (ByteView&)*base_view;
        PreReplayed pre(nm);
        if (ctx->last_runs.size() != nm) ctx->last_runs.assign(nm, 0);
        ctx->wave_off.assign(nm, 0);
        if (ctx->wave_pred.size() != nm) ctx->wave_pred.assign(nm, 0);
        std::vector<std::thread> wave_threads(nm);
        std::vector<int> wave_rc(nm, SX_OK);
        std::vector<char> threaded(nm, 0);
        struct Joiner {
            std::vector<std::thread>& t;
            ~Joiner() { for (auto& x : t) if (x.joinable()) x.join(); }
        } joiner{ wave_threads };
        const uint64_t defer_all = nm >= 2 ? (result_stays_on_device(ctx, job) ? 1 : ctx->sw.defer_min_bytes) : 0;
        if (nm >= 2 && ctx->sw.wave_threads) {
            if (ctx->wave_density.size() != nm) ctx->wave_density.assign(nm, 0.0);
            for (size_t k = 0; k < nm; k++) {
                const bool unscanned = k < not_scanned.size() && not_scanned[k];
                if (ctx->missions[k].host_sequential() || !unscanned || !wave_replay_wanted(ctx, job, k, len)) continue;
                threaded[k] = 1;
                ctx->stats.bytes_scanned += len;
                wave_threads[k] = std::thread([ctx, k, &early_view, &job, &pre, &wave_rc, defer_all]() {
                    (void)hipSetDevice(ctx->device);
                    wave_rc[k] = wave_replay_mission(ctx, k, early_view, job, &pre.per[k], &pre.ends[k], defer_all, true);
                });
            }
        }
        std::vector<size_t> order2;
        for (size_t oi = 0; oi < nm; oi++) if (!threaded[(size_t)order[oi]]) order2.push_back((size_t)order[oi]);
        for (size_t oi = 0; oi < nm; oi++) if (threaded[(size_t)order[oi]]) order2.push_back((size_t)order[oi]);
        for (size_t oi = 0; oi < nm; oi++) {
            const size_t k = order2[oi];
            std::vector<RunList> one;
            int rc = SX_OK;
            const bool unscanned = k < not_scanned.size() && not_scanned[k];
            bool replayed = false;
            if (threaded[k]) {
                wave_threads[k].join();
                rc = wave_rc[k];
                if (rc == SX_WAVE_FALLBACK) {
                    ctx->wave_off[k] = 1; ctx->wave_pred[k] = 0;
                    ctx->stats.bytes_scanned -= len;
                    rc = SX_OK;
                } else if (rc != SX_OK) return rc;
                else replayed = true;
            }
            if (replayed) {
                one.assign(1, RunList{});
                one[0].n = len / 16; one[0].skipped = true; one[0].complete = true;
            } else if (ctx->missions[k].host_sequential()) {
                one.assign(1, RunList{});
                one[0].complete = true;
            } else if (unscanned && wave_replay_wanted(ctx, job, k, len)) {
                one.assign(1, RunList{});
                one[0].n = len / 16; one[0].skipped = true; one[0].complete = true;
                ctx->stats.bytes_scanned += len;
            } else {
                if (unscanned) {
                    ctx->wave_pred[k] = 0;
                    rc = stage_a_launch(ctx, { (int)k }, d_bytes, len, { parity[k] }, { minc[k] }, slot);
                    if (rc != SX_OK) return rc;
                }
                rc = stage_a_finish(ctx, { (int)k }, d_bytes, len, { parity[k] }, { minc[k] }, slot, &one, true, &job);
            }
            if (rc != SX_OK) return rc;
            (*runs)[k] = std::move(one[0]);
            if (!(*runs)[k].own.empty()) (*runs)[k].use_own();
            ctx->last_runs[k] = (*runs)[k].size();
            const bool last_mission = oi + 1 == nm;
            bool next_queued = false;
            auto queue_next = [&]() -> int {
                if (!last_mission || !after_last_finish || next_queued) return SX_OK;
                next_queued = true;
                return after_last_finish();
            };
            if (!(*runs)[k].skipped && (rc = queue_next()) != SX_OK) return rc;
            if (replayed) { pre.done[k] = 1; if ((rc = queue_next()) != SX_OK) return rc; continue; }
            if (device_replay_wanted(ctx, job, k, (*runs)[k].size())) {
                SX_TL("mission %zu: device replay begins (%zu runs)", k, (*runs)[k].size());
                rc = device_replay_mission(ctx, k, early_view, job, (*runs)[k], &pre.per[k], &pre.ends[k], defer_all);
                SX_TL("mission %zu: device replay done", k);
                if (rc == SX_NEED_RUNS) {
                    ctx->wave_off[k] = 1;
                    rc = stage_a_launch(ctx, { (int)k }, d_bytes, len, { parity[k] }, { minc[k] }, slot);
                    if (rc == SX_OK) rc = stage_a_finish(ctx, { (int)k }, d_bytes, len, { parity[k] }, { minc[k] }, slot, &one, true, nullptr);
                    if (rc != SX_OK) return rc;
                    (*runs)[k] = std::move(one[0]);
                    if (!(*runs)[k].own.empty()) (*runs)[k].use_own();
                    ctx->last_runs[k] = (*runs)[k].size();
                    if ((rc = queue_next()) != SX_OK) return rc;
                    if (!device_replay_wanted(ctx, job, k, (*runs)[k].size())) continue;
                    rc = device_replay_mission(ctx, k, early_view, job, (*runs)[k], &pre.per[k], &pre.ends[k], defer_all);
                }
                if (rc != SX_OK) return rc;
                pre.done[k] = 1;
            }
            if ((rc = queue_next()) != SX_OK) return rc;
        }
        SX_TL("all missions finished / replayed on the device");
        if (host_bytes) return replay_all(ctx, host_view, job, *runs, into, ends, &pre);
        SparseDeviceBytes view(ctx, d_bytes, len);
        bool base_is_enough = false;
        int rc = download_for_replay(ctx, d_bytes, len, runs, &view, job, &pre.done, &base_is_enough);
        if (rc != SX_OK) return rc;
        return replay_all(ctx, base_is_enough ? (ByteView&)*base_view : (ByteView&)view, job, *runs, into, ends, &pre);
    }
};

int scan_common(sx_ctx* ctx, const uint8_t* host_bytes, const uint8_t* d_bytes, uint64_t len, int file_id,
                       int is_last, sx_result** out, uint32_t slice_base0, sx_result* append_to) {
    const double t_begin = now_ms();
    g_tl_on = ctx->sw.timeline; g_tl_t0 = t_begin;
    SX_TL("scan_common: %llu bytes", (unsigned long long)len);
    const size_t nm = ctx->missions.size();
    ctx->dev_epoch->fetch_add(1);
    ctx->shard_runs_valid = false;
    std::vector<uint64_t> stream0(nm);
    for (size_t k = 0; k < nm; k++) stream0[k] = ctx->states[k].stream_bytes;
    std::vector<int> order;
    mission_order(ctx, &order);
    const uint64_t seq_piece = ctx->host_only ? len : seq_piece_bytes(ctx, len);
    const bool seq = seq_piece < len;
    const uint64_t piece = seq ? seq_piece : piece_bytes(ctx, len);
    const uint64_t n_pieces = len ? (len + piece - 1) / piece : 1;
    ctx->single_piece = n_pieces == 1 && !append_to;
    const uint64_t merged0 = ctx->merged_out_bytes;
    int entry_rc = SX_OK;
    auto make = [&](uint64_t p) {
        BufferScan b;
        const uint64_t off = p * piece;
        b.host_bytes = host_bytes ? host_bytes + off : nullptr;
        b.d_bytes = d_bytes + off;
        b.len = std::min(piece, len - off);
        b.order = order;
        b.whole = true;
        b.slot = (int)(p & 1);
        for (size_t k = 0; k < nm; k++) {
            uint32_t ep = (uint32_t)((stream0[k] + off) & 1);
            if (ctx->missions[k].is_dbcs()) {
                uint32_t ep_replay = 0;
                entry_rc = std::min(entry_rc, entry_param(ctx, k, &ctx->states[k].decoder, b.host_bytes, b.d_bytes, b.len, 0, &ep, &ep_replay));
                ctx->missions[k].buf_entry_skip = ep_replay;
            }
            b.parity.push_back(ep);
            b.minc.push_back(ctx->missions[k].long_run);
        }
        return b;
    };
    ResultHolder res;
    int rc = SX_OK;
    if (seq) {
        ctx->merge_async = true;
        ctx->stats.seq_pieces += n_pieces;
        for (uint64_t p = 0; p < n_pieces; p++) {
            BufferScan b = make(p);
            if (entry_rc != SX_OK) return sync_streams_and_return(ctx, entry_rc);
            if ((rc = b.launch(ctx)) != SX_OK) return sync_streams_and_return(ctx, rc);
            if ((rc = b.fetch_base(ctx)) != SX_OK) return sync_streams_and_return(ctx, rc);
            ReplayJob job = whole_chunk_job(ctx, b.len, file_id, is_last != 0 && p + 1 == n_pieces);
            job.d_bytes = b.d_bytes;
            job.slice_base = slice_base0 + (uint32_t)(p * piece / kInputBufLen);
            std::vector<RunList> runs;
            rc = b.finish_and_replay(ctx, job, nullptr, &runs, append_to ? &append_to->r : &res.r->r, nullptr);
            if (rc != SX_OK) return sync_streams_and_return(ctx, rc);
        }
        ctx->merge_async = false;
        if ((rc = merge_drain(ctx)) != SX_OK) return sync_streams_and_return(ctx, rc);
        if (len) ctx->out_density = (double)(ctx->merged_out_bytes - merged0) / (double)len;
        ctx->stats.total_ms = now_ms() - t_begin;
        if (!append_to) *out = res.release();
        return SX_OK;
    }
    std::vector<BufferScan> pieces;
    for (uint64_t p = 0; p < n_pieces; p++) pieces.push_back(make(p));
    if (entry_rc != SX_OK) return entry_rc;
    uint64_t launched = 0;
    for (; launched < std::min<uint64_t>(2, n_pieces); launched++)
        if ((rc = pieces[launched].launch(ctx)) != SX_OK) return sync_streams_and_return(ctx, rc);
    SX_TL("scans queued");
    if ((rc = pieces[0].fetch_base(ctx)) != SX_OK) return sync_streams_and_return(ctx, rc);
    SX_TL("base fetched");
    for (uint64_t p = 0; p < n_pieces; p++) {
        BufferScan& b = pieces[p];
        if (p > 0 && (rc = b.fetch_base(ctx)) != SX_OK) return sync_streams_and_return(ctx, rc);
        ReplayJob job = whole_chunk_job(ctx, b.len, file_id, is_last != 0 && p + 1 == n_pieces);
        job.d_bytes = b.d_bytes;
        job.slice_base = slice_base0 + (uint32_t)(p * piece / kInputBufLen);
        std::vector<RunList> runs;
        rc = b.finish_and_replay(ctx, job,
                                 [&]() -> int { return launched < n_pieces ? pieces[launched++].launch(ctx) : SX_OK; },
                                 &runs, append_to ? &append_to->r : &res.r->r, nullptr);
        if (rc != SX_OK) return sync_streams_and_return(ctx, rc);
    }
    if (len) ctx->out_density = (double)(ctx->merged_out_bytes - merged0) / (double)len;
    ctx->stats.total_ms = now_ms() - t_begin;
    SX_TL("scan_common done");
    if (!append_to) *out = res.release();
    return SX_OK;
}


int shard_common(sx_ctx* ctx, const uint8_t* host_bytes, const uint8_t* d_bytes,
                        const sx_run* const* given_runs, const uint64_t* given_n, uint64_t buf_off, uint64_t buf_len,
                        uint64_t own_lo, uint64_t own_hi, const uint64_t* start_at, uint64_t file_stream_off, int file_id,
                        int reuse_runs, sx_result** out, uint64_t* end_pos) {
    if (!out || !end_pos || (buf_off % kInputBufLen) != 0 || own_lo < buf_off || own_hi < own_lo || own_hi > buf_off + buf_len) {
        ctx->err = "bad shard geometry"; return SX_E_INVALID;
    }
    ctx->sharded_call = true;
    const size_t nm = ctx->missions.size();
    const double t_begin = now_ms();
    for (const Mission& m : ctx->missions)
        if (m.host_sequential()) {
            ctx->err = "an ISO-2022-JP mission cannot be sharded: the character set in force at a shard start depends on every escape "
                       "sequence in front of it (its stage B is one sequential pass)";
            return SX_E_INVALID;
        }
    for (const Mission& m : ctx->missions)
        if (m.c.chars_min_nb == 0 && buf_off != 0) {
            ctx->err = "a mission with chars_min_nb 0 cannot be sharded: its state at a shard start cannot be derived from the bytes "
                       "in front of it (stage B runs as one sequential pass for it)";
            return SX_E_INVALID;
        }
    if (buf_off > 0) {
        bool any = false;
        for (const Mission& m : ctx->missions) any = any || m.is_dbcs();
        if (any) {
            const uint64_t front = own_lo - buf_off;
            std::vector<char> found(nm, 0);
            std::vector<uint8_t> tmp;
            auto all_found = [&]() { for (size_t k = 0; k < nm; k++) if (ctx->missions[k].is_dbcs() && !found[k]) return false; return true; };
            for (uint64_t at = 0; at < front && !all_found(); at += 65536) {
                const uint64_t n = std::min<uint64_t>(65536, front - at);
                const uint8_t* s = host_bytes ? host_bytes + at : nullptr;
                if (!s) {
                    tmp.resize(n);
                    HIP_TRY(ctx, hipMemcpy(tmp.data(), d_bytes + at, n, hipMemcpyDeviceToHost));
                    s = tmp.data();
                }
                for (size_t k = 0; k < nm; k++) {
                    const Mission& m = ctx->missions[k];
                    if (!m.is_dbcs() || found[k]) continue;
                    const int enc = m.c.encoding;
                    const bool two = enc_family((uint32_t)enc) == 4;
                    for (uint64_t i = 0; i < n; i++)
                        if (!(two ? dbcs_may_be_pending_after<4>(s[i], enc) : dbcs_may_be_pending_after<5>(s[i], enc))) { found[k] = 1; break; }
                }
            }
            if (!all_found()) {
                ctx->err = "no byte outside the lead range between the buffer start and own_lo: the token grid of a double-byte "
                           "mission is unknown there; repeat with a larger halo in front";
                return SX_E_HALO;
            }
        }
    }
    if (given_runs) {
        ctx->shard_runs.assign(nm, RunList{});
        for (size_t k = 0; k < nm; k++) ctx->shard_runs[k].assign(given_runs[k], given_runs[k] + given_n[k]);
    }
    const void* buf_id = d_bytes ? (const void*)d_bytes : (const void*)host_bytes;
    const bool same_buffer = ctx->shard_runs_valid && ctx->shard_runs_off == buf_off && ctx->shard_runs_len == buf_len && ctx->shard_runs_ptr == buf_id;
    const bool scan_now = !given_runs && !(reuse_runs && same_buffer);
    if (given_runs || scan_now) ctx->shard_runs_valid = false;
    BufferScan b;
    {
        int rc = set_entry_params(ctx, buf_off == 0, host_bytes, d_bytes, buf_len, file_stream_off + buf_off, &b.parity);
        if (rc != SX_OK) return rc;
    }
    if (scan_now) {
        b.host_bytes = host_bytes; b.d_bytes = d_bytes; b.len = buf_len; mission_order(ctx, &b.order); b.slot = 0;
        for (size_t k = 0; k < nm; k++) b.minc.push_back(ctx->missions[k].long_run);
        int rc = b.launch(ctx);
        if (rc == SX_OK) rc = b.fetch_base(ctx);
        if (rc != SX_OK) return sync_streams_and_return(ctx, rc);
    }

    ReplayJob job;
    job.len = buf_len; job.file_id = file_id; job.is_last = false;
    job.hi = own_hi - buf_off;
    job.commit_state = job.hi >= buf_len;
    job.slice_base = (uint32_t)(buf_off / kInputBufLen);
    for (size_t k = 0; k < nm; k++) {
        uint64_t lo = own_lo;
        if (start_at && start_at[k] > lo) lo = start_at[k];
        if (lo > own_hi) lo = own_hi;
        job.lo.push_back(lo - buf_off);
        job.entry_exact.push_back(buf_off == 0 && lo == 0);
        job.consumed0.push_back(ctx->missions[k].c.counter_offset + file_stream_off + buf_off);
        job.stream0.push_back(file_stream_off + buf_off);
    }
    job.d_bytes = d_bytes;
    int rc;
    ResultHolder res;
    std::vector<uint64_t> ends(nm, 0);
    if (scan_now) {
        ctx->shard_runs_valid = false;
        rc = b.finish_and_replay(ctx, job, nullptr, &ctx->shard_runs, &res.r->r, ends.data());
        if (rc != SX_OK) return sync_streams_and_return(ctx, rc);
        ctx->shard_runs_valid = true; ctx->shard_runs_off = buf_off; ctx->shard_runs_len = buf_len; ctx->shard_runs_ptr = buf_id;
    } else if (host_bytes) {
        HostBytes view(host_bytes);
        rc = replay_all(ctx, view, job, ctx->shard_runs, &res.r->r, ends.data());
    } else {
        SparseDeviceBytes view(ctx, d_bytes, buf_len);
        rc = download_for_replay(ctx, d_bytes, buf_len, &ctx->shard_runs, &view, job);
        if (rc != SX_OK) return rc;
        rc = replay_all(ctx, view, job, ctx->shard_runs, &res.r->r, ends.data());
    }
    if (rc == SX_OK) *out = res.release();
    for (size_t k = 0; k < nm; k++) end_pos[k] = buf_off + ends[k];
    ctx->stats.total_ms = now_ms() - t_begin;
    return rc;
}


}
```

stringsext_amd/csrc/sx_sort.hip:

```cpp
#include <hip/hip_runtime.h>
#include <cstring>
#include <cstdio>
#include <cstdlib>
#include <ctime>
#include <rocprim/device/device_radix_sort.hpp>
#include <rocprim/device/device_scan.hpp>
#include <rocprim/iterator/counting_iterator.hpp>
#include <rocprim/iterator/transform_iterator.hpp>

#include "sx_device.hpp"

namespace sx {

__global__ __launch_bounds__(256) void split_records_kernel(const DevRun* recs, uint32_t n, uint64_t* keys, uint64_t* vals) {
    const uint32_t i = blockIdx.x * 256u + threadIdx.x;
    if (i >= n) return;
    const DevRun r = recs[i];
    const bool invalid = r.len == kRecInvalidLen && r.chars_flags == kRecInvalidFlags;
    keys[i] = invalid ? ~0ull : r.start;
    vals[i] = ((uint64_t)r.chars_flags << 32) | r.len;
}
__global__ __launch_bounds__(256) void join_records_kernel(const uint64_t* keys, const uint64_t* vals, uint32_t n, DevRun* out) {
    const uint32_t i = blockIdx.x * 256u + threadIdx.x;
    if (i >= n) return;
// ... 347 lines not shown
        hipLaunchKernelGGL(merge_range_kernel, dim3(1), dim3(64), 0, stream, L, T, rg);
        const uint64_t nb_threads = ((uint64_t)T + 1) * (uint64_t)n_missions;
        hipLaunchKernelGGL(merge_bounds_kernel, dim3((unsigned)((nb_threads + 255) / 256)), dim3(256), 0, stream, L, T, rg, bounds);
        for (int m = 0; m < n_missions; m++)
            if (nf[m])
                hipLaunchKernelGGL(merge_place_kernel, dim3((unsigned)((nf[m] + 255) / 256)), dim3(256), 0, stream, L, m, T, rg, bounds, (void*)out_f, packed, src);
        if (ordered) {
            uint8_t* rest = (uint8_t*)src + ((size_t)n * 8 + 255) / 256 * 256;
            return order_part_strings(out, n, packed, src, out_a, rest, scratch_bytes - (size_t)(rest - (uint8_t*)scratch), stream);
        }
        return hipGetLastError();
    }
    sx_finding* all = (sx_finding*)base;
    uint64_t* k0 = (uint64_t*)(base + ((n * sizeof(sx_finding) + 255) & ~(size_t)255));
    uint64_t* v0 = k0 + n;
    uint64_t* k1 = v0 + n;
    uint64_t* v1 = k1 + n;
    uint8_t* tmp = (uint8_t*)(((uintptr_t)(v1 + n) + 255) & ~(uintptr_t)255);
    size_t tmp_bytes = scratch_bytes - (size_t)(tmp - (uint8_t*)scratch);
    uint64_t fb = 0, ab = 0;
    for (int m = 0; m < n_missions; m++) {
        if (nf[m]) {
            hipLaunchKernelGGL(merge_gather_in_kernel, dim3((unsigned)((nf[m] + 255) / 256)), dim3(256), 0, stream, f[m], nf[m],
                               (uint32_t)ab - off0[m], fb, all, k0, v0);
            hipError_t e = hipMemcpyAsync(out_a + ab, a[m], nb[m], hipMemcpyDeviceToDevice, stream);
            if (e != hipSuccess) return e;
        }
        fb += nf[m]; ab += nb[m];
    }
    hipError_t e = rocprim::radix_sort_pairs(tmp, tmp_bytes, k0, k1, v0, v1, (size_t)n, 0, 64, stream);
    if (e != hipSuccess) return e;
    hipLaunchKernelGGL(merge_gather_out_kernel, dim3((unsigned)((n + 255) / 256)), dim3(256), 0, stream, all, v1, n, out_f);
    return hipGetLastError();
}

typedef unsigned int copy_v4u __attribute__((ext_vector_type(4)));
template <bool NT>
__global__ __launch_bounds__(1024) void copy_bytes_kernel(copy_v4u* __restrict__ dst, const copy_v4u* __restrict__ src, uint64_t n16,
                                                          uint8_t* dst_tail, const uint8_t* src_tail, uint32_t n_tail) {
    const uint64_t per = (n16 + gridDim.x - 1) / gridDim.x;
    const uint64_t begin = per * blockIdx.x, end = begin + per < n16 ? begin + per : n16;
    const uint64_t stride = blockDim.x;
    uint64_t i = begin + threadIdx.x;
    n16 = end;
    for (; i + 3 * stride < n16; i += 4 * stride) {
        const copy_v4u a = __builtin_nontemporal_load(src + i), b = __builtin_nontemporal_load(src + i + stride);
        const copy_v4u c = __builtin_nontemporal_load(src + i + 2 * stride), d = __builtin_nontemporal_load(src + i + 3 * stride);
        if (NT) {
            __builtin_nontemporal_store(a, dst + i); __builtin_nontemporal_store(b, dst + i + stride);
            __builtin_nontemporal_store(c, dst + i + 2 * stride); __builtin_nontemporal_store(d, dst + i + 3 * stride);
        } else { dst[i] = a; dst[i + stride] = b; dst[i + 2 * stride] = c; dst[i + 3 * stride] = d; }
    }
    for (; i < n16; i += stride) dst[i] = src[i];
    if (blockIdx.x == 0 && threadIdx.x < n_tail) dst_tail[threadIdx.x] = src_tail[threadIdx.x];
}
__global__ __launch_bounds__(64) void small_copy_kernel(uint32_t* dst, const uint32_t* src, uint32_t n_words) {
    const uint32_t t = blockIdx.x * 64 + threadIdx.x, nt = gridDim.x * 64;
    if ((((uintptr_t)dst | (uintptr_t)src) & 15) == 0) {
        const uint32_t n4 = n_words / 4;
        for (uint32_t i = t; i < n4; i += nt) ((uint4*)dst)[i] = ((const uint4*)src)[i];
        for (uint32_t i = n4 * 4 + t; i < n_words; i += nt) dst[i] = src[i];
    } else for (uint32_t i = t; i < n_words; i += nt) dst[i] = src[i];
}
hipError_t launch_small_copy(void* pinned_dst, const void* dev_src, size_t bytes, hipStream_t stream) {
    if (!bytes) return hipSuccess;
    if ((((uintptr_t)pinned_dst | (uintptr_t)dev_src | bytes) & 3) != 0 || bytes > (1u << 20)) return hipErrorInvalidValue;
    const unsigned blocks = bytes <= 16384 ? 1u : (bytes <= 131072 ? 2u : 4u);
    hipLaunchKernelGGL(small_copy_kernel, dim3(blocks), dim3(64), 0, stream, (uint32_t*)pinned_dst, (const uint32_t*)dev_src, (uint32_t)(bytes / 4));
    return hipGetLastError();
}
hipError_t launch_copy_bytes(void* dst, const void* src, uint64_t bytes, uint32_t workgroups, hipStream_t stream, int threads, bool nt) {
    if (!bytes) return hipSuccess;
    if ((((uintptr_t)dst | (uintptr_t)src) & 15) != 0) return hipErrorInvalidValue;
    const uint64_t n16 = bytes / 16;
    if (nt)
        hipLaunchKernelGGL(copy_bytes_kernel<true>, dim3(workgroups ? workgroups : 2), dim3((unsigned)threads), 0, stream, (copy_v4u*)dst, (const copy_v4u*)src, n16,
                           (uint8_t*)dst + n16 * 16, (const uint8_t*)src + n16 * 16, (uint32_t)(bytes - n16 * 16));
    else
        hipLaunchKernelGGL(copy_bytes_kernel<false>, dim3(workgroups ? workgroups : 2), dim3((unsigned)threads), 0, stream, (copy_v4u*)dst, (const copy_v4u*)src, n16,
                           (uint8_t*)dst + n16 * 16, (const uint8_t*)src + n16 * 16, (uint32_t)(bytes - n16 * 16));
    return hipGetLastError();
}

__global__ __launch_bounds__(64) void merge_cuts_kernel(const sx_finding* f, uint64_t n, uint64_t nb, const uint64_t* cuts, uint32_t n_cuts,
                                                        uint64_t* idx, uint64_t* off) {
    const uint32_t j = blockIdx.x * 64u + threadIdx.x;
    if (j >= n_cuts) return;
    const uint64_t c = cuts[j];
    uint64_t lo = 0, hi = n;
    while (lo < hi) {
        const uint64_t mid = lo + (hi - lo) / 2;
        if (f[mid].position < c) lo = mid + 1; else hi = mid;
    }
    idx[j] = lo;
    off[j] = lo < n ? f[lo].str_off : nb;
}
hipError_t launch_merge_cuts(const sx_finding* f, uint64_t n, uint64_t nb, const uint64_t* cuts, uint32_t n_cuts, uint64_t* idx,
                             uint64_t* off, hipStream_t stream) {
    if (n_cuts == 0) return hipSuccess;
    hipLaunchKernelGGL(merge_cuts_kernel, dim3((n_cuts + 63) / 64), dim3(64), 0, stream, f, n, nb, cuts, n_cuts, idx, off);
    return hipGetLastError();
}

}
```

stringsext_amd/csrc/sx_stage_a.cpp:

```cpp
#include "sx_ctx.hpp"

using namespace sx;

namespace sx {

static bool large_regions_fit(uint64_t len, uint64_t n_regions, uint32_t cap) {
    const uint64_t slots = n_regions * cap;
    return slots < (1ull << 31) && slots * sizeof(DevRun) <= std::max<uint64_t>(256ull << 20, len / 2);
}

static uint32_t subchunk_bytes(const sx_ctx* ctx) {
    const uint32_t sub = ctx->opt.subchunk_bytes ? ctx->opt.subchunk_bytes : 256u * 1024u;
    return std::max<uint32_t>(kTileBytes, sub / kTileBytes * kTileBytes);
}

static bool fusion_allowed(const sx_ctx* ctx) {
    return !(ctx->opt.flags & (SX_OPT_NO_FUSED_SCAN | SX_OPT_MISSION_STREAMS)) && !ctx->sw.mission_streams && ctx->sw.fused && ctx->sw.scan_warm < 0;
}

ScanParams scan_params(const sx_ctx* ctx, int mission, const ScanSlot& s, const uint8_t* d_bytes, uint64_t len,
                       uint32_t parity, uint64_t min_chars) {
    const Mission& m = ctx->missions[(size_t)mission];
    ScanParams p = m.proto;
    p.data = d_bytes; p.len = len; p.subchunk = subchunk_bytes(ctx); p.parity = parity;
    p.pair_lut = ctx->dev[(size_t)mission].d_pair_lut;
    if (p.gb4) {
        p.gb_ranges = ctx->dev[(size_t)mission].d_table ? ctx->dev[(size_t)mission].d_table + kGbN : nullptr;
        p.ubf = m.c.ubf;
        if (!p.gb_ranges) p.gb4 = 0;
    }
    p.wave_prio = ctx->sw.scan_prio;
    p.min_chars = (uint32_t)std::min<uint64_t>(min_chars, kRecCharsMask);
    if (p.min_chars == 0) p.min_chars = 1;
    p.cand_bytes = std::min<uint32_t>(p.min_chars * (m.is_utf16() ? 2u : 1u), 14u);
    {
        uint32_t have = 1;
        for (int i = 0; i < 5; i++) {
            const uint32_t sh = have < p.cand_bytes ? std::min(have, p.cand_bytes - have) : 0;
            p.cand_sh[i] = sh;
            have += sh;
        }
    }
    p.capacity = s.capacity; p.recs = s.d_recs; p.counters = s.d_counters;
    p.region_cap = s.region_cap; p.region_counts = s.d_cnt; p.grid_flags = s.d_grid;
    unsigned occ = ctx->scan_blocks_per_cu;
    p.persistent = (occ >= 1 && occ < 8) ? occ * ctx->n_cus : 0u;
    return p;
}

int stage_a_launch(sx_ctx* ctx, const std::vector<int>& which, const uint8_t* d_bytes, uint64_t len,
                   const std::vector<uint32_t>& parity, const std::vector<uint64_t>& min_chars, int si) {
    if (len == 0) return SX_OK;
    for (size_t k = 0; k < which.size(); k++) {
        MissionDev& d = ctx->dev[(size_t)which[k]];
        ScanSlot& s = d.slot[si];
        if (s.free_pending) { HIP_TRY(ctx, hipStreamWaitEvent(d.stream, s.ev_free, 0)); s.free_pending = false; }
        {
            const uint32_t sub = subchunk_bytes(ctx);
            const uint64_t n_regions = (len + sub - 1) / sub;
            if (ctx->dense.size() != ctx->missions.size()) ctx->dense.assign(ctx->missions.size(), 0);
            s.region_cap = 0; s.n_regions = n_regions;
            const uint32_t dn = ctx->dense[(size_t)which[k]];
            const uint32_t want_cap = dn > 1 ? dn : (dn == 0 ? ctx->region_cap : 0u);
            if (ctx->region_cap && want_cap &&
                (dn > 1 ? large_regions_fit(len, n_regions, want_cap) : n_regions * want_cap < (1ull << 28))) {
                s.region_cap = want_cap;
                int rc = ensure_capacity(ctx, s, (uint32_t)(n_regions * s.region_cap));
                if (rc != SX_OK && dn > 1) {
                    (void)hipGetLastError();
                    ctx->dense[(size_t)which[k]] = 1;
                    s.region_cap = 0;
                    rc = SX_OK;
                }
                if (rc != SX_OK) return rc;
                if (s.region_cap == 0) goto launch;
                if (s.cnt_cap < n_regions) {
                    if (s.d_cnt) HIP_TRY(ctx, hipFree(s.d_cnt));
                    s.d_cnt = nullptr; s.cnt_cap = 0;
                    HIP_TRY(ctx, hipMalloc((void**)&s.d_cnt, (n_regions + n_regions / 4 + 64) * 4));
                    s.cnt_cap = n_regions + n_regions / 4 + 64;
                }
            }
        }
    launch:
        const bool dbcs = ctx->missions[(size_t)which[k]].is_dbcs();
        if (dbcs) {
            const uint32_t sub = subchunk_bytes(ctx);
            const uint64_t n_sub = (len + sub - 1) / sub;
            if (s.grid_cap < n_sub) {
                if (s.d_grid) HIP_TRY(ctx, hipFree(s.d_grid));
                s.d_grid = nullptr; s.grid_cap = 0;
                HIP_TRY(ctx, hipMalloc((void**)&s.d_grid, (n_sub + n_sub / 4 + 64) * 4));
                s.grid_cap = n_sub + n_sub / 4 + 64;
            }
        }
    }
    std::vector<char> fused(which.size(), 0);
    std::vector<ScanParams> params(which.size());
    for (size_t k = 0; k < which.size(); k++)
        params[k] = scan_params(ctx, which[k], ctx->dev[(size_t)which[k]].slot[si], d_bytes, len, parity[k], min_chars[k]);
// ... 250 lines not shown
```

stringsext_amd/csrc/sx_stage_b.cpp:

```cpp
#include "sx_ctx.hpp"

using namespace sx;

namespace sx {

static inline uint64_t win_start_h(uint64_t p, size_t W) {
    const uint64_t s0 = p / kInputBufLen * kInputBufLen;
    return s0 + (p - s0) / W * W;
}

bool device_replay_wanted(const sx_ctx* ctx, const ReplayJob& job, size_t k, size_t n_runs) {
    if (!job.d_bytes || ctx->host_only || job.is_last || ctx->missions[k].host_sequential()) return false;
    if (ctx->opt.flags & SX_OPT_HOST_REPLAY) return false;
    if (ctx->missions[k].q > 255) return false;
    if (ctx->missions[k].c.chars_min_nb == 0) return false;
    if (ctx->sw.host_replay) return false;
    if (wave_replay_wanted(ctx, job, k, n_runs)) return true;
    return (ctx->opt.flags & SX_OPT_DEVICE_REPLAY) || ctx->sw.device_replay || n_runs >= 4096;
}

struct Slab {
    size_t i0 = 0, i1 = 0;
    bool first = true, last = true;
    int out_slot = 5;
// ... 721 lines not shown
    std::atomic<size_t> next{ 0 };
    std::vector<double> task_ms(tasks.size(), 0.0);
    auto worker = [&]() {
        for (;;) {
            const size_t t = next.fetch_add(1);
            if (t >= tasks.size()) break;
            const size_t k = tasks[t].first, p = tasks[t].second;
            const double tt0 = now_ms();
            replay_part(ctx->missions[k], ctx->states[k], job.consumed0[k], job.stream0[k], bytes, job.len, job.file_id,
                        job.is_last, runs[k].data(), runs[k].size(), bounds[k][p], bounds[k][p + 1],
                        p == 0 && job.entry_exact[k], &parts[k][p]);
            task_ms[t] = now_ms() - tt0;
        }
    };
    const size_t nw = host_runs < 2048 ? 1 : std::min<size_t>(nthreads, tasks.size());
    if (nw <= 1) worker();
    else {
        std::vector<std::thread> th;
        for (size_t i = 0; i < nw; i++) th.emplace_back(worker);
        for (auto& t : th) t.join();
    }
    const double t_parts = now_ms();
    std::vector<MissionFindings> per(nm);
    std::vector<uint64_t> ends(nm, 0);
    for (size_t k = 0; k < nm; k++) {
        if (on_device[k] == 2) { per[k] = std::move(pre->per[k]); pre->per[k].ext = {}; ends[k] = pre->ends[k]; }
        else if (on_device[k] == 3) {
            int rc = host_sequential_mission(ctx, k, bytes, job, &per[k]);
            if (rc != SX_OK) return rc;
            ends[k] = job.len;
        } else if (on_device[k]) {
            int rc = device_replay_mission(ctx, k, bytes, job, runs[k], &per[k], &ends[k], 0);
            if (rc != SX_OK) return rc;
        }
    }
    auto stitch = [&](size_t k) {
        if (on_device[k]) return;
        ScannerState st = ctx->states[k];
        replay_stitch(ctx->missions[k], st, job.consumed0[k], job.stream0[k], bytes, job.len, job.file_id, job.is_last,
                      runs[k].data(), runs[k].size(), parts[k], &per[k], nthreads, &ends[k]);
        if (job.commit_state) ctx->states[k] = st;
        if (job.slice_base) for (auto& f : per[k].v) f.slice_index += job.slice_base;
    };
    if (nm == 1) stitch(0);
    else {
        std::vector<std::thread> th;
        for (size_t k = 0; k < nm; k++) th.emplace_back(stitch, k);
        for (auto& t : th) t.join();
    }
    if (end_pos) for (size_t k = 0; k < nm; k++) end_pos[k] = ends[k];
    const double t_stitch = now_ms();
    SX_TL("replay_all: host parts + stitch done");
    const size_t count_before = into->count();
    {
        int rc = device_merge(ctx, job, per, into);
        if (rc != SX_OK) return rc;
    }
    SX_TL("replay_all: device_merge done");
    merge_findings(per, ctx->pool, into, ctx->sw.host_merge_seg_bytes);
    SX_TL("replay_all: merge_findings done");
    if (ctx->sw.timing) {
        double mx = 0, sum = 0;
        for (double v : task_ms) { sum += v; mx = std::max(mx, v); }
        fprintf(stderr, "[sx] replay: parts %.2f ms (%zu tasks, %zu workers; task sum %.1f max %.1f ms), stitch %.2f ms, merge %.2f ms, "
                        "on-demand fetches so far %llu\n", t_parts - t0, tasks.size(), nw, sum, mx, t_stitch - t_parts,
                now_ms() - t_stitch, (unsigned long long)ctx->ondemand_fetches);
    }
    for (auto& mf : per) ctx->stats.replay_bytes += mf.replay_bytes;
    ctx->stats.findings += into->count() - count_before;
    ctx->stats.replay_ms += now_ms() - t0;
    return SX_OK;
}

ReplayJob whole_chunk_job(sx_ctx* ctx, uint64_t len, int file_id, bool is_last) {
    ReplayJob j;
    const size_t nm = ctx->missions.size();
    j.len = len; j.file_id = file_id; j.is_last = is_last; j.hi = len;
    j.lo.assign(nm, 0); j.entry_exact.assign(nm, 1);
    for (size_t k = 0; k < nm; k++) { j.consumed0.push_back(ctx->states[k].consumed_bytes); j.stream0.push_back(ctx->states[k].stream_bytes); }
    return j;
}


int download_for_replay(sx_ctx* ctx, const uint8_t* d_bytes, uint64_t len,
                               const std::vector<RunList>* runs_opt, SparseDeviceBytes* view,
                               const ReplayJob& job, const std::vector<char>* skip, bool* used_base) {
    const size_t nm = runs_opt ? ctx->missions.size() : 0;
    static const std::vector<RunList> no_runs;
    const std::vector<RunList>& runs = runs_opt ? *runs_opt : no_runs;
    if (used_base) *used_base = false;
        const double t0 = now_ms();
        std::vector<std::pair<uint64_t, uint64_t>> rg;
        rg.emplace_back(0, std::min<uint64_t>(len, 64 * 1024));
        if (len > 64 * 1024) rg.emplace_back(len - 64 * 1024, len);
        for (size_t k = 0; k < nm; k++) {
            if ((skip && (*skip)[k]) || ctx->missions[k].host_sequential() || device_replay_wanted(ctx, job, k, runs[k].size())) continue;
            HIP_TRY(ctx, runs[k].wait());
            const size_t before = rg.size();
            unsigned want_parts = (unsigned)std::min<uint64_t>(replay_threads(ctx), std::max<uint64_t>(1, runs[k].size() / 512));
            if (ctx->missions[k].c.chars_min_nb == 0) want_parts = 1;
            replay_ranges(ctx->missions[k], ctx->states[k], len, runs[k].data(), runs[k].size(), want_parts, &rg);
            if (!std::is_sorted(rg.begin() + before, rg.end())) std::sort(rg.begin() + before, rg.end());
            std::inplace_merge(rg.begin(), rg.begin() + before, rg.end());
        }
        const double t_rg = now_ms();
        std::vector<std::pair<uint64_t, uint64_t>> mg;
        mg.reserve(rg.size());
        for (auto& r : rg) {
            if (!mg.empty() && r.first <= mg.back().second) mg.back().second = std::max(mg.back().second, r.second);
            else mg.push_back(r);
        }
        if (used_base) {
            bool inside = true;
            for (auto& r : mg)
                inside = inside && (r.second <= std::min<uint64_t>(len, 64 * 1024) || (len > 64 * 1024 && r.first >= len - 64 * 1024));
            if (inside) { *used_base = true; return SX_OK; }
        }
        std::vector<uint64_t> seg_src, seg_dst;
        std::vector<uint32_t> seg_len;
        uint64_t total = 0;
        for (auto& r : mg)
            for (uint64_t a = r.first; a < r.second; a += 65536) {
                const uint64_t n = std::min<uint64_t>(65536, r.second - a);
                seg_src.push_back(a); seg_dst.push_back(total); seg_len.push_back((uint32_t)n);
                total += n;
            }
        const double t_seg = now_ms();
        if (total) {
            hipStream_t s = ctx->dev[0].stream_b;
            const size_t ns = seg_src.size();
            const uint64_t seg_bytes = ns * (8 + 8 + 4) + 64;
            int rc2 = ensure_pinned(ctx, total + 64);
            if (rc2 != SX_OK) return rc2;
            rc2 = ensure_scratch(ctx, total + seg_bytes + 256);
            if (rc2 != SX_OK) return rc2;
            uint8_t* d_out = ctx->d_scratch;
            uint64_t* d_src = (uint64_t*)(ctx->d_scratch + ((total + 255) & ~255ull));
            uint64_t* d_dst = d_src + ns;
            uint32_t* d_len = (uint32_t*)(d_dst + ns);
            HIP_TRY(ctx, hipMemcpyAsync(d_src, seg_src.data(), ns * 8, hipMemcpyHostToDevice, s));
            HIP_TRY(ctx, hipMemcpyAsync(d_dst, seg_dst.data(), ns * 8, hipMemcpyHostToDevice, s));
            HIP_TRY(ctx, hipMemcpyAsync(d_len, seg_len.data(), ns * 4, hipMemcpyHostToDevice, s));
            HIP_TRY(ctx, launch_gather(d_bytes, d_out, d_src, d_dst, d_len, (uint32_t)ns, s));
            HIP_TRY(ctx, hipMemcpyAsync(ctx->h_pin, d_out, total, hipMemcpyDeviceToHost, s));
            HIP_TRY(ctx, hipStreamSynchronize(s));
            uint64_t off = 0;
            for (auto& r : mg) {
                if (runs_opt) view->add(r.first, r.second, ctx->h_pin + off);
                else view->add_copy(r.first, r.second, ctx->h_pin + off);
                off += r.second - r.first;
            }
        }
        ctx->stats.d2h_ms += now_ms() - t0;
        if (ctx->sw.timing)
            fprintf(stderr, "[sx] sparse download: ranges %.2f ms, sort+merge+segments %.2f ms (%zu ranges, %zu segs), gather+d2h %.2f ms (%.1f MB)\n",
                    t_rg - t0, t_seg - t_rg, mg.size(), seg_src.size(), now_ms() - t_seg, total / 1e6);
    return SX_OK;
}

}
```

stringsext_amd/csrc/sx_switches.cpp:

```cpp
#include "sx_switches.hpp"

#include <stdio.h>
#include <stdlib.h>

#include <algorithm>

namespace sx {

static bool present(const char* name) { return getenv(name) != nullptr; }
static bool on_unless_0(const char* name) { const char* e = getenv(name); return !(e && !atoi(e)); }
static bool on_if_nonzero(const char* name) { const char* e = getenv(name); return e && atoi(e); }
static int int_or(const char* name, int unset) { const char* e = getenv(name); return e ? atoi(e) : unset; }
static int64_t i64_or(const char* name, int64_t unset) { const char* e = getenv(name); return e ? (int64_t)atoll(e) : unset; }
static int clamped_or(const char* name, int lo, int hi, int unset) { const char* e = getenv(name); return e ? std::max(lo, std::min(hi, atoi(e))) : unset; }
static uint64_t u64_at_least(const char* name, uint64_t lo, uint64_t unset) { const char* e = getenv(name); return e ? std::max<uint64_t>(lo, (uint64_t)atoll(e)) : unset; }

Switches Switches::from_env() {
    Switches s;
    if (const char* e = getenv("SX_PIN_FLAGS")) s.pin_flags = (int64_t)(unsigned)strtoul(e, nullptr, 0);
    s.small_copy = on_unless_0("SX_SMALL_COPY");
    if (const char* e = getenv("SX_REPLAY_THREADS")) s.replay_threads = (int)std::max(1u, std::min(256u, (unsigned)atoi(e)));
    s.result_on_device = on_if_nonzero("SX_RESULT_ON_DEVICE");
    s.scan_blocks_per_cu = int_or("SX_SCAN_BLOCKS_PER_CU", s.scan_blocks_per_cu);
    if (const char* e = getenv("SX_REGION_CAP")) s.region_cap = (int64_t)(uint32_t)atoi(e);
    s.scan_cus = clamped_or("SX_SCAN_CUS", 1, INT32_MAX, s.scan_cus);
    if (const char* e = getenv("SX_PRIO")) s.prio_n = std::max(0, sscanf(e, "%d,%d", &s.prio_scan, &s.prio_post));
    s.mission_streams = present("SX_MISSION_STREAMS");
    s.scan_prio = (uint32_t)int_or("SX_SCAN_PRIO", (int)s.scan_prio);
    s.fused = on_unless_0("SX_FUSED");
    s.fused_prefilter = int_or("SX_FUSED_PREFILTER", s.fused_prefilter);
    s.scan_warm = clamped_or("SX_SCAN_WARM", 0, INT32_MAX, s.scan_warm);
    s.no_large_regions = present("SX_NO_LARGE_REGIONS");
    s.device_join_min = (uint32_t)int_or("SX_DEVICE_JOIN_MIN", (int)s.device_join_min);
    s.no_pieces = present("SX_NO_PIECES");
    s.probe_rot = (uint32_t)int_or("SX_PROBE_ROT", (int)s.probe_rot);
    s.host_replay = present("SX_HOST_REPLAY");
    s.device_replay = present("SX_DEVICE_REPLAY");
    s.host_stitch = present("SX_HOST_STITCH");
    s.no_replay_skip = present("SX_NO_REPLAY_SKIP");
    s.no_grid_bound = present("SX_NO_GRID_BOUND");
    s.no_replay_cache = present("SX_NO_REPLAY_CACHE");
    s.max_region_windows = (uint32_t)clamped_or("SX_MAX_REGION_WINDOWS", 1, INT32_MAX, (int)s.max_region_windows);
    s.replay_cache_mib = i64_or("SX_REPLAY_CACHE_MIB", s.replay_cache_mib);
    s.fast_replay = on_unless_0("SX_FAST_REPLAY");
    s.count_waves = int_or("SX_COUNT_WAVES", s.count_waves);
    s.stitch_block = clamped_or("SX_STITCH_BLOCK", 0, INT32_MAX, s.stitch_block);
    s.slabs = clamped_or("SX_SLABS", 1, 64, s.slabs);
    s.replay_copy_wgs = int_or("SX_REPLAY_COPY_WGS", s.replay_copy_wgs);
    s.host_merge = present("SX_HOST_MERGE");
    s.packed = on_unless_0("SX_PACKED");
    s.merge_part_mib = u64_at_least("SX_MERGE_PART_MIB", 1, s.merge_part_mib);
    s.merge_part_findings = u64_at_least("SX_MERGE_PART_FINDINGS", 1024, s.merge_part_findings);
    s.merge_copy_wgs = int_or("SX_MERGE_COPY_WGS", s.merge_copy_wgs);
    s.merge_copy_nt = int_or("SX_MERGE_COPY_NT", s.merge_copy_nt);
    s.merge_copy_threads = clamped_or("SX_MERGE_COPY_THREADS", 64, 1024, s.merge_copy_threads);
    s.host_merge_seg_bytes = u64_at_least("SX_HOST_MERGE_SEG_BYTES", 1, s.host_merge_seg_bytes);
    s.splice_seg_bytes = u64_at_least("SX_SPLICE_SEG_BYTES", 1, s.splice_seg_bytes);
    s.piece_mib = i64_or("SX_PIECE_MIB", s.piece_mib);
    s.seq_piece_kib = i64_or("SX_SEQ_PIECE_KIB", s.seq_piece_kib);
    s.seq_piece_mib = i64_or("SX_SEQ_PIECE_MIB", s.seq_piece_mib);
    s.debug_entry = present("SX_DEBUG_ENTRY");
    s.busiest_last = int_or("SX_BUSIEST_LAST", s.busiest_last);
    if (const char* e = getenv("SX_DEFER_MIN_BYTES")) s.defer_min_bytes = (uint64_t)atoll(e);
    s.wave_threads = on_unless_0("SX_WAVE_THREADS");
    s.timeline = int_or("SX_TIMELINE", s.timeline);
    s.timing = present("SX_TIMING");
    s.timing2 = present("SX_TIMING2");
    if (const char* e = getenv("SX_WAVE_REPLAY")) s.wave_replay = atoi(e) != 0;
    s.wave_keep_scan = present("SX_WAVE_KEEP_SCAN");
    if (const char* e = getenv("SX_WAVE_BYTES_PER_RUN")) s.wave_bytes_per_run = (uint64_t)atoll(e);
    s.wave_stream_prio = int_or("SX_WAVE_STREAM_PRIO", s.wave_stream_prio);
    s.wave_batches = clamped_or("SX_WAVE_BATCHES", 1, 64, s.wave_batches);
    s.wave_slabs = clamped_or("SX_WAVE_SLABS", 1, 64, s.wave_slabs);
    s.wave_lut = on_if_nonzero("SX_WAVE_LUT");
    s.wave_desc = on_unless_0("SX_WAVE_DESC");
    s.wave_desc_cap = clamped_or("SX_WAVE_DESC_CAP", 1, INT32_MAX, s.wave_desc_cap);
    s.wave_fail = present("SX_WAVE_FAIL");
    if (const char* e = getenv("SX_WAVE_REPAIR")) s.wave_repair = atoi(e) ? std::max(1, atoi(e)) : 0;
    s.wave_same = on_unless_0("SX_WAVE_SAME");
    if (const char* e = getenv("SX_SCAN_STREAM_MIB")) s.scan_stream_mib = (uint64_t)atoll(e);
    s.ingest_mmap = present("SX_INGEST_MMAP");
    return s;
}

}
```

stringsext_amd/csrc/sx_switches.hpp:

```cpp
#pragma once
#include <stdint.h>

namespace sx {

struct Switches {
    int64_t pin_flags = -1;
    bool small_copy = true;
    int replay_threads = 0;
    bool result_on_device = false;
    int scan_blocks_per_cu = -1;
    int64_t region_cap = -1;
    int scan_cus = 0;
    int prio_n = -1, prio_scan = 0, prio_post = 0;
    bool mission_streams = false;
    uint32_t scan_prio = 0;
    bool fused = true;
    int fused_prefilter = -1;
    int scan_warm = -1;
    bool no_large_regions = false;
    uint32_t device_join_min = 65536;
    bool no_pieces = false;
    uint32_t probe_rot = 0;
    bool host_replay = false;
    bool device_replay = false;
    bool host_stitch = false;
    bool no_replay_skip = false;
    bool no_grid_bound = false;
    bool no_replay_cache = false;
    uint32_t max_region_windows = 0;
    int64_t replay_cache_mib = -1;
    bool fast_replay = true;
    int count_waves = 4;
    int stitch_block = 0;
    int slabs = 0;
    int replay_copy_wgs = 0;
    bool host_merge = false;
    bool packed = true;
    uint64_t merge_part_mib = 0;
    uint64_t merge_part_findings = 0;
    int merge_copy_wgs = -1;
    int merge_copy_nt = 1;
    int merge_copy_threads = 512;
    uint64_t host_merge_seg_bytes = 0;
    uint64_t splice_seg_bytes = 0;
    int64_t piece_mib = -1;
    int64_t seq_piece_kib = -1;
    int64_t seq_piece_mib = -1;
    bool debug_entry = false;
    int busiest_last = 0;
    uint64_t defer_min_bytes = 256ull << 20;
    bool wave_threads = true;
    int timeline = 0;
    bool timing = false;
    bool timing2 = false;
    int wave_replay = -1;
    bool wave_keep_scan = false;
    uint64_t wave_bytes_per_run = 0;
    int wave_stream_prio = -1;
    int wave_batches = 0;
    int wave_slabs = 0;
    bool wave_lut = false;
    bool wave_desc = true;
    int wave_desc_cap = 0;
    bool wave_fail = false;
    int wave_repair = -1;
    bool wave_same = true;
    uint64_t scan_stream_mib = 0;
    bool ingest_mmap = false;

    static Switches from_env();
};

}
```

Measured before the change: 3985.

## Prefetch base edge bytes asynchronously via tiled gather into pinned host memory

Replaces the per-piece synchronous base fetch with one asynchronous gather kernel that writes the head and tail 64 KiB of every piece straight into a pinned host buffer. An event is recorded, and the sparse view waits on it lazily the first time it is read, so the base download overlaps with the scan launches. The gather kernel is rewritten to use 1 KiB tiles with an inline segment table and aligned destinations. The automatic piece-splitting condition is also generalised to use the fused-launch check and tunable thresholds. The cost is more complexity: lazy synchronisation through an atomic and a mutex, and a kernel that writes directly into host memory.

```diff
diff --git a/include/stringsext_amd.h b/include/stringsext_amd.h
--- a/include/stringsext_amd.h
+++ b/include/stringsext_amd.h
@@ -277,6 +277,8 @@
 int sx_device_free(sx_ctx* ctx, void* device_ptr);
 int sx_device_upload(sx_ctx* ctx, void* device_dst, const void* host_src, uint64_t bytes);
 int sx_device_download(sx_ctx* ctx, void* host_dst, const void* device_src, uint64_t bytes);
+int sx_device_download_ranges(sx_ctx* ctx, void* host_dst, const void* device_src, const uint64_t* lo, const uint64_t* hi,
+                              uint64_t n_ranges);
 int sx_device_read_bandwidth(sx_ctx* ctx, const void* device_bytes, uint64_t len, int repeats,
                              double* gbytes_per_s);
 
diff --git a/stringsext_amd/__init__.py b/stringsext_amd/__init__.py
--- a/stringsext_amd/__init__.py
+++ b/stringsext_amd/__init__.py
@@ -29,7 +29,7 @@
            "sx_result_count", "sx_result_segments", "sx_result_segment", "sx_result_segment_device", "sx_result_findings", "sx_result_arena",
            "sx_result_free", "sx_print_findings", "sx_print_findings_device", "sx_result_select_device",
            "sx_select_set_create", "sx_select_set_info_get", "sx_select_set_free", "sx_result_select_set_device", "sx_get_stats", "sx_free", "sx_fill_background_device",
-           "sx_device_alloc", "sx_device_free", "sx_device_upload", "sx_device_download",
+           "sx_device_alloc", "sx_device_free", "sx_device_upload", "sx_device_download", "sx_device_download_ranges",
            "sx_device_read_bandwidth"]
 
 
@@ -237,6 +237,7 @@
     L.sx_device_free.argtypes = [vp, vp]
     L.sx_device_upload.argtypes = [vp, vp, cp, u64]
     L.sx_device_download.argtypes = [vp, vp, vp, u64]
+    L.sx_device_download_ranges.argtypes = [vp, vp, vp, C.POINTER(u64), C.POINTER(u64), u64]
     L.sx_device_read_bandwidth.argtypes = [vp, vp, u64, C.c_int, C.POINTER(C.c_double)]
     _lib = L
     return L
@@ -550,6 +551,14 @@
         self._chk(lib().sx_device_download(self.h, b, dptr, nbytes))
         return b.raw
 
+    def download_ranges(self, dptr, ranges):
+        n = len(ranges)
+        lo = (C.c_uint64 * max(n, 1))(*[r[0] for r in ranges])
+        hi = (C.c_uint64 * max(n, 1))(*[r[1] for r in ranges])
+        b = C.create_string_buffer(max(1, sum(r[1] - r[0] for r in ranges)))
+        self._chk(lib().sx_device_download_ranges(self.h, b, dptr, lo, hi, n))
+        return b.raw[:sum(r[1] - r[0] for r in ranges)]
+
     def fill_background(self, dptr, first_index, nbytes, seed=0x5EED5EED5EED5EED):
         self._chk(lib().sx_fill_background_device(self.h, dptr, first_index, nbytes, seed))
 
diff --git a/stringsext_amd/csrc/sx_api.cpp b/stringsext_amd/csrc/sx_api.cpp
--- a/stringsext_amd/csrc/sx_api.cpp
+++ b/stringsext_amd/csrc/sx_api.cpp
@@ -97,6 +97,16 @@
     bytes += bytes / 4 + (1u << 20);
     HIP_TRY(ctx, hipHostMalloc((void**)&ctx->h_pin2, bytes, hipHostMallocNonCoherent));
     ctx->h_pin2_cap = bytes;
+    return SX_OK;
+}
+int ensure_base(sx_ctx* ctx, uint64_t bytes) {
+    if (!ctx->ev_base) HIP_TRY(ctx, hipEventCreateWithFlags(&ctx->ev_base, hipEventDisableTiming));
+    if (ctx->h_base_cap >= bytes) return SX_OK;
+    if (ctx->h_base) HIP_TRY(ctx, hipHostFree(ctx->h_base));
+    ctx->h_base = nullptr; ctx->h_base_cap = 0;
+    bytes += bytes / 4 + (1u << 16);
+    HIP_TRY(ctx, hipHostMalloc((void**)&ctx->h_base, bytes, hipHostMallocNonCoherent));
+    ctx->h_base_cap = bytes;
     return SX_OK;
 }
 int ensure_scratch(sx_ctx* ctx, uint64_t bytes) {
@@ -398,6 +408,8 @@
         if (ctx->d_scratch) (void)hipFree(ctx->d_scratch);
         if (ctx->h_pin) (void)hipHostFree(ctx->h_pin);
         if (ctx->h_pin2) (void)hipHostFree(ctx->h_pin2);
+        if (ctx->h_base) (void)hipHostFree(ctx->h_base);
+        if (ctx->ev_base) (void)hipEventDestroy(ctx->ev_base);
     }
     delete ctx;
 }
@@ -877,6 +889,27 @@
     return SX_OK;
 }
 
+int sx_device_download_ranges(sx_ctx* ctx, void* host_dst, const void* device_src, const uint64_t* lo, const uint64_t* hi, uint64_t n_ranges) {
+    if (!ctx || ctx->host_only) return SX_E_STATE;
+    if (n_ranges && (!host_dst || !lo || !hi)) { ctx->err = "null argument"; return SX_E_INVALID; }
+    HIP_TRY(ctx, hipSetDevice(ctx->device));
+    std::vector<std::pair<uint64_t, uint64_t>> rg;
+    for (uint64_t i = 0; i < n_ranges; i++) {
+        if (hi[i] < lo[i]) { ctx->err = "a range ends in front of its start"; return SX_E_INVALID; }
+        rg.emplace_back(lo[i], hi[i]);
+    }
+    std::vector<uint64_t> at;
+    uint64_t total = 0;
+    const int rc = gather_to_pinned(ctx, (const uint8_t*)device_src, rg, &at, &total);
+    if (rc != SX_OK) return rc;
+    uint8_t* out = (uint8_t*)host_dst;
+    for (uint64_t i = 0; i < n_ranges; i++) {
+        memcpy(out, ctx->h_pin + at[i], hi[i] - lo[i]);
+        out += hi[i] - lo[i];
+    }
+    return SX_OK;
+}
+
 int sx_device_read_bandwidth(sx_ctx* ctx, const void* device_bytes, uint64_t len, int repeats, double* gbytes_per_s) {
     if (!ctx || ctx->host_only || !gbytes_per_s || repeats == 0) return SX_E_STATE;
     HIP_TRY(ctx, hipSetDevice(ctx->device));
diff --git a/stringsext_amd/csrc/sx_ctx.hpp b/stringsext_amd/csrc/sx_ctx.hpp
--- a/stringsext_amd/csrc/sx_ctx.hpp
+++ b/stringsext_amd/csrc/sx_ctx.hpp
@@ -179,6 +179,8 @@
     uint8_t* h_pin = nullptr;   uint64_t h_pin_cap = 0;
     uint8_t* h_pin2 = nullptr;  uint64_t h_pin2_cap = 0;
     uint8_t* d_scratch = nullptr; uint64_t d_scratch_cap = 0;
+    uint8_t* h_base = nullptr;  uint64_t h_base_cap = 0;
+    hipEvent_t ev_base = nullptr;
 };
 
 #define HIP_TRY(ctx, expr)                                                                     \
@@ -195,6 +197,7 @@
 class SparseDeviceBytes : public ByteView {
 public:
     SparseDeviceBytes(sx_ctx* ctx, const uint8_t* d_base, uint64_t len = 0) : ctx_(ctx), d_base_(d_base), len_(len) {}
+    void wait_for(hipEvent_t ready) { ready_ = ready; pending_.store(true, std::memory_order_release); }
     void add(uint64_t lo, uint64_t hi, const uint8_t* p) { segs_.push_back({ lo, hi, p }); }
     void add_copy(uint64_t lo, uint64_t hi, const uint8_t* p) {
         owned_.emplace_back(p, p + (hi - lo));
@@ -202,6 +205,7 @@
     }
     bool empty() const { return segs_.empty(); }
     const uint8_t* span(uint64_t off, size_t n, size_t* hint) override {
+        if (pending_.load(std::memory_order_acquire)) settle();
         size_t a = *hint < segs_.size() ? *hint : 0;
         if (!(a < segs_.size() && segs_[a].lo <= off)) a = 0;
         size_t steps = 0;
@@ -238,7 +242,15 @@
     }
 
 private:
+    void settle() {
+        std::lock_guard<std::mutex> g(mu_);
+        if (!pending_.load(std::memory_order_acquire)) return;
+        if (hipEventSynchronize(ready_) != hipSuccess) segs_.clear();
+        pending_.store(false, std::memory_order_release);
+    }
     struct Seg { uint64_t lo, hi; const uint8_t* p; };
+    hipEvent_t ready_ = nullptr;
+    std::atomic<bool> pending_{ false };
     sx_ctx* ctx_;
     const uint8_t* d_base_;
     uint64_t len_ = 0;
@@ -251,6 +263,7 @@
 
 int ensure_pinned(sx_ctx* ctx, uint64_t bytes);
 int ensure_pinned2(sx_ctx* ctx, uint64_t bytes);
+int ensure_base(sx_ctx* ctx, uint64_t bytes);
 int read_back_sync(sx_ctx* ctx, sx::MissionDev& d, hipStream_t s, void* host_dst, const void* dev_src, size_t bytes);
 int read_back_async(sx_ctx* ctx, hipStream_t s, void* pinned_dst, const void* dev_src, size_t bytes);
 int ensure_scratch(sx_ctx* ctx, uint64_t bytes);
@@ -263,6 +276,7 @@
 
 ScanParams scan_params(const sx_ctx* ctx, int mission, const ScanSlot& s, const uint8_t* d_bytes, uint64_t len,
                        uint32_t parity, uint64_t min_chars);
+bool fused_launch_expected(const sx_ctx* ctx);
 int stage_a_launch(sx_ctx* ctx, const std::vector<int>& which, const uint8_t* d_bytes, uint64_t len,
                    const std::vector<uint32_t>& parity, const std::vector<uint64_t>& min_chars, int si);
 struct ReplayJob;
@@ -316,6 +330,9 @@
                         const ReplayJob& job, const std::vector<char>* skip = nullptr,
                         bool* used_base = nullptr);
 
+int gather_to_pinned(sx_ctx* ctx, const uint8_t* d_bytes, const std::vector<std::pair<uint64_t, uint64_t>>& rg, std::vector<uint64_t>* at,
+                     uint64_t* total);
+
 struct ResultHolder {
     sx_result* r = new sx_result();
     ~ResultHolder() { delete r; }
diff --git a/stringsext_amd/csrc/sx_device.hpp b/stringsext_amd/csrc/sx_device.hpp
--- a/stringsext_amd/csrc/sx_device.hpp
+++ b/stringsext_amd/csrc/sx_device.hpp
@@ -236,7 +236,14 @@
 hipError_t launch_fill_background(uint8_t* dst, uint64_t first_index, uint64_t len, uint64_t seed,
                                   hipStream_t stream);
 hipError_t launch_read_sum(const uint8_t* src, uint64_t len, uint64_t* out, hipStream_t stream, uint32_t subchunk = 0, uint32_t rot = 0);
-hipError_t launch_gather(const uint8_t* src, uint8_t* dst, const uint64_t* seg_src, const uint64_t* seg_dst,
-                         const uint32_t* seg_len, uint32_t n, hipStream_t stream);
+constexpr uint32_t kGatherTile = 1024;
+constexpr uint32_t kGatherInline = 16;
+struct GatherSeg {
+    uint64_t src, dst, len;
+    uint64_t tile0;
+};
+inline uint64_t gather_dst_offset(uint64_t dst_end, uint64_t src_addr) { return dst_end + ((src_addr - dst_end) & 15u); }
+uint64_t gather_plan(GatherSeg* segs, uint32_t n, const uint8_t* dst);
+hipError_t launch_gather(const uint8_t* src, uint8_t* dst, const GatherSeg* segs, uint32_t n, uint64_t n_tiles, hipStream_t stream);
 
 }
diff --git a/stringsext_amd/csrc/sx_kernels.hip b/stringsext_amd/csrc/sx_kernels.hip
--- a/stringsext_amd/csrc/sx_kernels.hip
+++ b/stringsext_amd/csrc/sx_kernels.hip
@@ -665,25 +665,4 @@
     return hipGetLastError();
 }
 
-__global__ __launch_bounds__(256) void gather_kernel(const uint8_t* src, uint8_t* dst, const u64* seg_src,
-                                                     const u64* seg_dst, const u32* seg_len, u32 n) {
-    u32 wave = (blockIdx.x * 256u + threadIdx.x) >> 6, lane = threadIdx.x & 63u;
-    u32 nw = (gridDim.x * 256u) >> 6;
-    for (u32 i = wave; i < n; i += nw) {
-        const uint8_t* s = src + seg_src[i];
-        uint8_t* d = dst + seg_dst[i];
-        u32 l = seg_len[i];
-        for (u32 k = lane; k < l; k += 64) d[k] = s[k];
-    }
-}
-
-hipError_t launch_gather(const uint8_t* src, uint8_t* dst, const u64* seg_src, const u64* seg_dst,
-                         const u32* seg_len, u32 n, hipStream_t stream) {
-    if (n == 0) return hipSuccess;
-    u32 blocks = (n + 3) / 4;
-    if (blocks > 256 * 8) blocks = 256 * 8;
-    hipLaunchKernelGGL(gather_kernel, dim3(blocks), dim3(256), 0, stream, src, dst, seg_src, seg_dst, seg_len, n);
-    return hipGetLastError();
-}
-
-}
+}
diff --git a/stringsext_amd/csrc/sx_schedule.cpp b/stringsext_amd/csrc/sx_schedule.cpp
--- a/stringsext_amd/csrc/sx_schedule.cpp
+++ b/stringsext_amd/csrc/sx_schedule.cpp
@@ -9,8 +9,10 @@
     uint64_t piece = 0;
     bool halves = false;
     if (ctx->sw.piece_mib >= 0) piece = (uint64_t)ctx->sw.piece_mib << 20;
-    else if (len >= (16ull << 30) && ctx->missions.size() >= 2 && !(ctx->opt.flags & (SX_OPT_NO_FUSED_SCAN | SX_OPT_MISSION_STREAMS | SX_OPT_RESULT_ON_DEVICE))) {
-        piece = ((len / 100) * 50 + kInputBufLen - 1) / kInputBufLen * kInputBufLen;
+    else if (len >= ((uint64_t)ctx->sw.piece_auto_min_mib << 20) && len >= 2 * kInputBufLen && !(ctx->opt.flags & SX_OPT_RESULT_ON_DEVICE) &&
+             fused_launch_expected(ctx)) {
+        const uint64_t share = ctx->sw.piece_tail_pct > 0 ? (len / 200) * (uint64_t)(100 - ctx->sw.piece_tail_pct) : (len / 100) * 50;
+        piece = (share + kInputBufLen - 1) / kInputBufLen * kInputBufLen;
         halves = true;
     }
     if (piece == 0 || (!halves && len < 2 * piece)) return len;
@@ -108,14 +110,6 @@
         return true;
     }
 
-    int fetch_base(sx_ctx* ctx) {
-        base_view.reset();
-        if (host_bytes) return SX_OK;
-        base_view.reset(new SparseDeviceBytes(ctx, d_bytes, len));
-        if (none_scanned(ctx)) return SX_OK;
-        ReplayJob none;
-        return download_for_replay(ctx, d_bytes, len, nullptr, base_view.get(), none);
-    }
     std::vector<char> not_scanned;
     int launch(sx_ctx* ctx) {
         not_scanned.assign(ctx->missions.size(), 0);
@@ -237,6 +231,50 @@
         return replay_all(ctx, base_is_enough ? (ByteView&)*base_view : (ByteView&)view, job, *runs, into, ends, &pre);
     }
 };
+
+static int prefetch_base(sx_ctx* ctx, BufferScan* const* bs, size_t n) {
+    struct Part { size_t b; uint64_t lo, hi, off; };
+    std::vector<Part> parts;
+    std::vector<GatherSeg> segs;
+    const uint8_t* src0 = nullptr;
+    for (size_t i = 0; i < n; i++) {
+        bs[i]->base_view.reset();
+        if (bs[i]->host_bytes) continue;
+        bs[i]->base_view.reset(new SparseDeviceBytes(ctx, bs[i]->d_bytes, bs[i]->len));
+        if (bs[i]->len && (!src0 || bs[i]->d_bytes < src0)) src0 = bs[i]->d_bytes;
+    }
+    uint64_t total = 0;
+    for (size_t i = 0; i < n; i++) {
+        const BufferScan& b = *bs[i];
+        if (b.host_bytes || b.len == 0) continue;
+        const uint64_t edge = 64 * 1024;
+        std::pair<uint64_t, uint64_t> rg[2] = { { 0, std::min<uint64_t>(b.len, edge) }, { b.len - std::min<uint64_t>(b.len, edge), b.len } };
+        size_t nr = 2;
+        if (rg[1].first <= rg[0].second) { rg[0].second = b.len; nr = 1; }
+        for (size_t r = 0; r < nr; r++) {
+            const uint64_t off = gather_dst_offset(total, (uint64_t)(uintptr_t)(b.d_bytes + rg[r].first));
+            parts.push_back({ i, rg[r].first, rg[r].second, off });
+            segs.push_back({ (uint64_t)(b.d_bytes - src0) + rg[r].first, off, rg[r].second - rg[r].first, 0 });
+            total = off + (rg[r].second - rg[r].first);
+        }
+    }
+    if (segs.empty()) return SX_OK;
+    const uint64_t tab_off = (total + 63) & ~63ull;
+    int rc = ensure_base(ctx, tab_off + segs.size() * sizeof(GatherSeg));
+    if (rc != SX_OK) return rc;
+    const uint64_t n_tiles = gather_plan(segs.data(), (uint32_t)segs.size(), ctx->h_base);
+    const GatherSeg* tab = segs.data();
+    if (segs.size() > kGatherInline) {
+        memcpy(ctx->h_base + tab_off, segs.data(), segs.size() * sizeof(GatherSeg));
+        tab = (const GatherSeg*)(ctx->h_base + tab_off);
+    }
+    hipStream_t s = ctx->dev[0].stream_b;
+    HIP_TRY(ctx, launch_gather(src0, ctx->h_base, tab, (uint32_t)segs.size(), n_tiles, s));
+    HIP_TRY(ctx, hipEventRecord(ctx->ev_base, s));
+    for (const Part& p : parts) bs[p.b]->base_view->add(p.lo, p.hi, ctx->h_base + p.off);
+    for (size_t i = 0; i < n; i++) if (bs[i]->base_view) bs[i]->base_view->wait_for(ctx->ev_base);
+    return SX_OK;
+}
 
 int scan_common(sx_ctx* ctx, const uint8_t* host_bytes, const uint8_t* d_bytes, uint64_t len, int file_id,
                        int is_last, sx_result** out, uint32_t slice_base0, sx_result* append_to) {
@@ -286,8 +324,11 @@
         for (uint64_t p = 0; p < n_pieces; p++) {
             BufferScan b = make(p);
             if (entry_rc != SX_OK) return sync_streams_and_return(ctx, entry_rc);
+            {
+                BufferScan* one = &b;
+                if ((rc = prefetch_base(ctx, &one, 1)) != SX_OK) return sync_streams_and_return(ctx, rc);
+            }
             if ((rc = b.launch(ctx)) != SX_OK) return sync_streams_and_return(ctx, rc);
-            if ((rc = b.fetch_base(ctx)) != SX_OK) return sync_streams_and_return(ctx, rc);
             ReplayJob job = whole_chunk_job(ctx, b.len, file_id, is_last != 0 && p + 1 == n_pieces);
             job.d_bytes = b.d_bytes;
             job.slice_base = slice_base0 + (uint32_t)(p * piece / kInputBufLen);
@@ -305,15 +346,18 @@
     std::vector<BufferScan> pieces;
     for (uint64_t p = 0; p < n_pieces; p++) pieces.push_back(make(p));
     if (entry_rc != SX_OK) return entry_rc;
+    {
+        std::vector<BufferScan*> all;
+        for (BufferScan& b : pieces) all.push_back(&b);
+        if ((rc = prefetch_base(ctx, all.data(), all.size())) != SX_OK) return sync_streams_and_return(ctx, rc);
+    }
+    SX_TL("base fetch queued");
     uint64_t launched = 0;
     for (; launched < std::min<uint64_t>(2, n_pieces); launched++)
         if ((rc = pieces[launched].launch(ctx)) != SX_OK) return sync_streams_and_return(ctx, rc);
     SX_TL("scans queued");
-    if ((rc = pieces[0].fetch_base(ctx)) != SX_OK) return sync_streams_and_return(ctx, rc);
-    SX_TL("base fetched");
     for (uint64_t p = 0; p < n_pieces; p++) {
         BufferScan& b = pieces[p];
-        if (p > 0 && (rc = b.fetch_base(ctx)) != SX_OK) return sync_streams_and_return(ctx, rc);
         ReplayJob job = whole_chunk_job(ctx, b.len, file_id, is_last != 0 && p + 1 == n_pieces);
         job.d_bytes = b.d_bytes;
         job.slice_base = slice_base0 + (uint32_t)(p * piece / kInputBufLen);
@@ -401,8 +445,9 @@
     if (scan_now) {
         b.host_bytes = host_bytes; b.d_bytes = d_bytes; b.len = buf_len; mission_order(ctx, &b.order); b.slot = 0;
         for (size_t k = 0; k < nm; k++) b.minc.push_back(ctx->missions[k].long_run);
-        int rc = b.launch(ctx);
-        if (rc == SX_OK) rc = b.fetch_base(ctx);
+        BufferScan* one = &b;
+        int rc = prefetch_base(ctx, &one, 1);
+        if (rc == SX_OK) rc = b.launch(ctx);
         if (rc != SX_OK) return sync_streams_and_return(ctx, rc);
     }
 
diff --git a/stringsext_amd/csrc/sx_sort.hip b/stringsext_amd/csrc/sx_sort.hip
--- a/stringsext_amd/csrc/sx_sort.hip
+++ b/stringsext_amd/csrc/sx_sort.hip
@@ -453,6 +453,64 @@
     return hipGetLastError();
 }
 
+struct GatherInlineTable { GatherSeg s[kGatherInline]; };
+__device__ __forceinline__ void gather_tile(const uint8_t* src, uint8_t* dst, const GatherSeg& g, uint64_t w, uint32_t lane) {
+    const uint8_t* s = src + g.src;
+    uint8_t* d = dst + g.dst;
+    const uint64_t da = (uint64_t)((uintptr_t)d & 15u);
+    const uint64_t v = (w - g.tile0) * kGatherTile + lane * 16u, lo = da, hi = da + g.len;
+    if (v >= hi || v + 16 <= lo) return;
+    if (v >= lo && v + 16 <= hi) {
+        copy_v4u x;
+        __builtin_memcpy(&x, s + (v - da), 16);
+        *(copy_v4u*)(d + (v - da)) = x;
+    } else {
+        const uint64_t a = v > lo ? v : lo, b = v + 16 < hi ? v + 16 : hi;
+        for (uint64_t k = a; k < b; k++) d[k - da] = s[k - da];
+    }
+}
+__global__ __launch_bounds__(256) void gather_ranges_kernel(const uint8_t* src, uint8_t* dst, const GatherSeg* segs, uint32_t n, uint64_t n_tiles) {
+    const uint64_t w = ((uint64_t)blockIdx.x * 256u + threadIdx.x) >> 6;
+    if (w >= n_tiles) return;
+    uint32_t lo = 0, hi = n;
+    while (hi - lo > 1) {
+        const uint32_t mid = lo + (hi - lo) / 2;
+        if (segs[mid].tile0 <= w) lo = mid; else hi = mid;
+    }
+    gather_tile(src, dst, segs[lo], w, threadIdx.x & 63u);
+}
+__global__ __launch_bounds__(256) void gather_ranges_inline_kernel(const uint8_t* src, uint8_t* dst, GatherInlineTable tab, uint32_t n, uint64_t n_tiles) {
+    const uint64_t w = ((uint64_t)blockIdx.x * 256u + threadIdx.x) >> 6;
+    if (w >= n_tiles) return;
+    GatherSeg g = tab.s[0];
+#pragma unroll
+    for (uint32_t i = 1; i < kGatherInline; i++)
+        if (i < n && tab.s[i].tile0 <= w) g = tab.s[i];
+    gather_tile(src, dst, g, w, threadIdx.x & 63u);
+}
+uint64_t gather_plan(GatherSeg* segs, uint32_t n, const uint8_t* dst) {
+    uint64_t tiles = 0;
+    for (uint32_t i = 0; i < n; i++) {
+        segs[i].tile0 = tiles;
+        const uint64_t da = ((uint64_t)(uintptr_t)dst + segs[i].dst) & 15u;
+        if (segs[i].len) tiles += (da + segs[i].len + kGatherTile - 1) / kGatherTile;
+    }
+    return tiles;
+}
+hipError_t launch_gather(const uint8_t* src, uint8_t* dst, const GatherSeg* segs, uint32_t n, uint64_t n_tiles, hipStream_t stream) {
+    if (n == 0 || n_tiles == 0) return hipSuccess;
+    const uint64_t blocks = (n_tiles + 3) / 4;
+    if (blocks > 0x7fffffffull) return hipErrorInvalidValue;
+    if (n <= kGatherInline) {
+        GatherInlineTable tab{};
+        for (uint32_t i = 0; i < n; i++) tab.s[i] = segs[i];
+        hipLaunchKernelGGL(gather_ranges_inline_kernel, dim3((unsigned)blocks), dim3(256), 0, stream, src, dst, tab, n, n_tiles);
+    } else {
+        hipLaunchKernelGGL(gather_ranges_kernel, dim3((unsigned)blocks), dim3(256), 0, stream, src, dst, segs, n, n_tiles);
+    }
+    return hipGetLastError();
+}
+
 __global__ __launch_bounds__(64) void merge_cuts_kernel(const sx_finding* f, uint64_t n, uint64_t nb, const uint64_t* cuts, uint32_t n_cuts,
                                                         uint64_t* idx, uint64_t* off) {
     const uint32_t j = blockIdx.x * 64u + threadIdx.x;
diff --git a/stringsext_amd/csrc/sx_stage_a.cpp b/stringsext_amd/csrc/sx_stage_a.cpp
--- a/stringsext_amd/csrc/sx_stage_a.cpp
+++ b/stringsext_amd/csrc/sx_stage_a.cpp
@@ -16,6 +16,23 @@
 
 static bool fusion_allowed(const sx_ctx* ctx) {
     return !(ctx->opt.flags & (SX_OPT_NO_FUSED_SCAN | SX_OPT_MISSION_STREAMS)) && !ctx->sw.mission_streams && ctx->sw.fused && ctx->sw.scan_warm < 0;
+}
+
+bool fused_launch_expected(const sx_ctx* ctx) {
+    if (!fusion_allowed(ctx)) return false;
+    const size_t nm = ctx->missions.size();
+    uint32_t used = 0;
+    for (size_t k = 0; k < nm; k++) {
+        const Mission& m = ctx->missions[k];
+        if (m.host_sequential()) continue;
+        if (k < ctx->wave_pred.size() && ctx->wave_pred[k] && m.wave_ok && !ctx->sw.wave_keep_scan && ctx->sw.wave_replay != 0) continue;
+        ScanParams p = m.proto;
+        p.region_cap = (ctx->dense.size() == nm && ctx->dense[k] == 1) ? 0u : ctx->region_cap;
+        p.persistent = (ctx->scan_blocks_per_cu >= 1 && ctx->scan_blocks_per_cu < 8) ? 1u : 0u;
+        const int sl = fused_slot_of(m.kind, p);
+        if (sl >= 0) used |= 1u << sl;
+    }
+    return __builtin_popcount(used) >= 2 || used == 1u;
 }
 
 ScanParams scan_params(const sx_ctx* ctx, int mission, const ScanSlot& s, const uint8_t* d_bytes, uint64_t len,
diff --git a/stringsext_amd/csrc/sx_stage_b.cpp b/stringsext_amd/csrc/sx_stage_b.cpp
--- a/stringsext_amd/csrc/sx_stage_b.cpp
+++ b/stringsext_amd/csrc/sx_stage_b.cpp
@@ -827,6 +827,44 @@
 }
 
 
+int gather_to_pinned(sx_ctx* ctx, const uint8_t* d_bytes, const std::vector<std::pair<uint64_t, uint64_t>>& rg, std::vector<uint64_t>* at,
+                     uint64_t* total_out) {
+    std::vector<GatherSeg> segs;
+    segs.reserve(rg.size());
+    at->clear();
+    uint64_t total = 0;
+    for (auto& r : rg) {
+        const uint64_t n = r.second > r.first ? r.second - r.first : 0;
+        const uint64_t off = gather_dst_offset(total, (uint64_t)(uintptr_t)(d_bytes + r.first));
+        segs.push_back({ r.first, off, n, 0 });
+        at->push_back(off);
+        total = off + n;
+    }
+    *total_out = total;
+    if (!total) return SX_OK;
+    if (segs.size() > 0xffffffffull) { ctx->set_err("too many byte ranges for one gather"); return SX_E_INVALID; }
+    hipStream_t s = ctx->dev[0].stream_b;
+    const size_t ns = segs.size();
+    const uint64_t tab_bytes = ns > kGatherInline ? ns * sizeof(GatherSeg) : 0;
+    const uint64_t h_tab = (total + 63) & ~63ull, d_tab = (total + 255) & ~255ull;
+    int rc = ensure_pinned(ctx, h_tab + tab_bytes + 64);
+    if (rc != SX_OK) return rc;
+    rc = ensure_scratch(ctx, d_tab + tab_bytes + 256);
+    if (rc != SX_OK) return rc;
+    uint8_t* d_out = ctx->d_scratch;
+    const uint64_t n_tiles = gather_plan(segs.data(), (uint32_t)ns, d_out);
+    const GatherSeg* tab = segs.data();
+    if (tab_bytes) {
+        memcpy(ctx->h_pin + h_tab, segs.data(), tab_bytes);
+        HIP_TRY(ctx, hipMemcpyAsync(d_out + d_tab, ctx->h_pin + h_tab, tab_bytes, hipMemcpyHostToDevice, s));
+        tab = (const GatherSeg*)(d_out + d_tab);
+    }
+    HIP_TRY(ctx, launch_gather(d_bytes, d_out, tab, (uint32_t)ns, n_tiles, s));
+    HIP_TRY(ctx, hipMemcpyAsync(ctx->h_pin, d_out, total, hipMemcpyDeviceToHost, s));
+    HIP_TRY(ctx, hipStreamSynchronize(s));
+    return SX_OK;
+}
+
 int download_for_replay(sx_ctx* ctx, const uint8_t* d_bytes, uint64_t len,
                                const std::vector<RunList>* runs_opt, SparseDeviceBytes* view,
                                const ReplayJob& job, const std::vector<char>* skip, bool* used_base) {
@@ -861,45 +899,21 @@
                 inside = inside && (r.second <= std::min<uint64_t>(len, 64 * 1024) || (len > 64 * 1024 && r.first >= len - 64 * 1024));
             if (inside) { *used_base = true; return SX_OK; }
         }
-        std::vector<uint64_t> seg_src, seg_dst;
-        std::vector<uint32_t> seg_len;
+        std::vector<uint64_t> at;
         uint64_t total = 0;
-        for (auto& r : mg)
-            for (uint64_t a = r.first; a < r.second; a += 65536) {
-                const uint64_t n = std::min<uint64_t>(65536, r.second - a);
-                seg_src.push_back(a); seg_dst.push_back(total); seg_len.push_back((uint32_t)n);
-                total += n;
-            }
         const double t_seg = now_ms();
-        if (total) {
-            hipStream_t s = ctx->dev[0].stream_b;
-            const size_t ns = seg_src.size();
-            const uint64_t seg_bytes = ns * (8 + 8 + 4) + 64;
-            int rc2 = ensure_pinned(ctx, total + 64);
+        {
+            const int rc2 = gather_to_pinned(ctx, d_bytes, mg, &at, &total);
             if (rc2 != SX_OK) return rc2;
-            rc2 = ensure_scratch(ctx, total + seg_bytes + 256);
-            if (rc2 != SX_OK) return rc2;
-            uint8_t* d_out = ctx->d_scratch;
-            uint64_t* d_src = (uint64_t*)(ctx->d_scratch + ((total + 255) & ~255ull));
-            uint64_t* d_dst = d_src + ns;
-            uint32_t* d_len = (uint32_t*)(d_dst + ns);
-            HIP_TRY(ctx, hipMemcpyAsync(d_src, seg_src.data(), ns * 8, hipMemcpyHostToDevice, s));
-            HIP_TRY(ctx, hipMemcpyAsync(d_dst, seg_dst.data(), ns * 8, hipMemcpyHostToDevice, s));
-            HIP_TRY(ctx, hipMemcpyAsync(d_len, seg_len.data(), ns * 4, hipMemcpyHostToDevice, s));
-            HIP_TRY(ctx, launch_gather(d_bytes, d_out, d_src, d_dst, d_len, (uint32_t)ns, s));
-            HIP_TRY(ctx, hipMemcpyAsync(ctx->h_pin, d_out, total, hipMemcpyDeviceToHost, s));
-            HIP_TRY(ctx, hipStreamSynchronize(s));
-            uint64_t off = 0;
-            for (auto& r : mg) {
-                if (runs_opt) view->add(r.first, r.second, ctx->h_pin + off);
-                else view->add_copy(r.first, r.second, ctx->h_pin + off);
-                off += r.second - r.first;
-            }
+        }
+        for (size_t i = 0; i < mg.size(); i++) {
+            if (runs_opt) view->add(mg[i].first, mg[i].second, ctx->h_pin + at[i]);
+            else view->add_copy(mg[i].first, mg[i].second, ctx->h_pin + at[i]);
         }
         ctx->stats.d2h_ms += now_ms() - t0;
         if (ctx->sw.timing)
-            fprintf(stderr, "[sx] sparse download: ranges %.2f ms, sort+merge+segments %.2f ms (%zu ranges, %zu segs), gather+d2h %.2f ms (%.1f MB)\n",
-                    t_rg - t0, t_seg - t_rg, mg.size(), seg_src.size(), now_ms() - t_seg, total / 1e6);
+            fprintf(stderr, "[sx] sparse download: ranges %.2f ms, sort+merge %.2f ms (%zu ranges), gather+d2h %.2f ms (%.1f MB)\n",
+                    t_rg - t0, t_seg - t_rg, mg.size(), now_ms() - t_seg, total / 1e6);
     return SX_OK;
 }
 
diff --git a/stringsext_amd/csrc/sx_switches.cpp b/stringsext_amd/csrc/sx_switches.cpp
--- a/stringsext_amd/csrc/sx_switches.cpp
+++ b/stringsext_amd/csrc/sx_switches.cpp
@@ -57,6 +57,8 @@
     s.host_merge_seg_bytes = u64_at_least("SX_HOST_MERGE_SEG_BYTES", 1, s.host_merge_seg_bytes);
     s.splice_seg_bytes = u64_at_least("SX_SPLICE_SEG_BYTES", 1, s.splice_seg_bytes);
     s.piece_mib = i64_or("SX_PIECE_MIB", s.piece_mib);
+    s.piece_auto_min_mib = std::max<int64_t>(0, i64_or("SX_PIECE_AUTO_MIN_MIB", s.piece_auto_min_mib));
+    s.piece_tail_pct = clamped_or("SX_PIECE_TAIL_PCT", 0, 49, s.piece_tail_pct);
     s.seq_piece_kib = i64_or("SX_SEQ_PIECE_KIB", s.seq_piece_kib);
     s.seq_piece_mib = i64_or("SX_SEQ_PIECE_MIB", s.seq_piece_mib);
     s.debug_entry = present("SX_DEBUG_ENTRY");
diff --git a/stringsext_amd/csrc/sx_switches.hpp b/stringsext_amd/csrc/sx_switches.hpp
--- a/stringsext_amd/csrc/sx_switches.hpp
+++ b/stringsext_amd/csrc/sx_switches.hpp
@@ -44,6 +44,8 @@
     uint64_t host_merge_seg_bytes = 0;
     uint64_t splice_seg_bytes = 0;
     int64_t piece_mib = -1;
+    int64_t piece_auto_min_mib = 16384;
+    int piece_tail_pct = 0;
     int64_t seq_piece_kib = -1;
     int64_t seq_piece_mib = -1;
     bool debug_entry = false;
```

New measurement: 3953. About the same (-0.8%).
